# distributed-information-bottleneck/distributed-information-bottleneck.github.io

Measured on AMD Instinct MI355X. Metric: DIB train samples/sec (fwd+KL+bwd+Adam), higher is better.
Workload: dtype f32; 1 GPU; BASELINE config 3: synthetic tabular, 2^20 rows x 64 scalar features resident in HBM, posenc [2,4,8,16], encoder [128,128], E=32, integration [256,256], out=1, BCE-from-logits, Adam; per_gpu_batch=65536, global_batch=65536, parallelism=dp1, rccl_ranks_joined=1, dataset_rows=1048576, params=2224897

## Files before the change

### distributed-information-bottleneck.github.io_amd/_lib.py

```python
from __future__ import annotations

import ctypes
import os
import shutil
import subprocess
from ctypes import POINTER, c_char_p, c_float, c_int, c_int32, c_int64, c_uint32, c_uint64, c_void_p

_HERE = os.path.dirname(os.path.abspath(__file__))
CSRC = os.path.join(_HERE, "csrc")
LIB_PATH = os.path.join(_HERE, "libdib_hip.so")
LIB_OVERRIDE = os.environ.get("DIB_LIB_PATH") or None
INCLUDE_DIR = os.path.join(os.path.dirname(_HERE), "include")


def _sources() -> list:
    out = []
    for root, _, names in os.walk(CSRC):
        out += [os.path.join(root, n) for n in names if n.endswith((".h", ".hip"))]
    out += [os.path.join(INCLUDE_DIR, n) for n in os.listdir(INCLUDE_DIR) if n.endswith(".h")]
    return sorted(out)


DIB_OK = 0
ABI_VERSION = 7
ACTIVATIONS = {None: 0, "linear": 0, "None": 0, "relu": 1, "leaky_relu": 2, "tanh": 3, "sigmoid": 4, "elu": 5,
               "softplus": 6}
ACT_LEAKY_RELU_01 = 7
LOSS_KINDS = {"bce_logits": 0, "bce": 1, "sparse_cce_logits": 2, "mse": 3}
WS_U, WS_PRED, WS_ENC_OUT, WS_G_U, WS_STEP_OUT, WS_G_PRED = range(6)
WS_ENC_H0, WS_INT_H0 = 16, 32
SYNC_WORDS = 1056
FWD_DETERMINISTIC, FWD_INFERENCE, FWD_DEFER_SUMS = 1, 2, 4
HEAD_DEFER_SUMS, HEAD_NO_GRAD, HEAD_DEFER_WGRAD = 1, 2, 4
BWD_INTEGRATION_DONE = 1
TAIL_FINALIZE, TAIL_KL, TAIL_LOSS, TAIL_ADAM, TAIL_BUMP, TAIL_METRICS, TAIL_SGD, TAIL_HEAD_WGRAD, TAIL_LOSS_HEAD = \
    1, 2, 4, 8, 16, 32, 64, 128, 256
SIMILARITIES = {"l2sq": 0, "l2": 1, "l1": 2, "linf": 3, "cosine": 4}


def _hipcc() -> str:
    for cand in (shutil.which("hipcc"), "/opt/rocm/bin/hipcc"):
        if cand and os.path.exists(cand):
            return cand
    raise RuntimeError("hipcc not found: cannot build libdib_hip.so")


def _stale() -> bool:
    if not os.path.exists(LIB_PATH):
        return True
    t = os.path.getmtime(LIB_PATH)
    return any(os.path.getmtime(p) > t for p in _sources())


def build_library(force: bool = False, verbose: bool = False) -> str:
    if not force and not _stale():
        return LIB_PATH
    cmd = [_hipcc(), "--offload-arch=gfx950", "-O3", "-std=c++17", "-shared", "-fPIC",
           os.path.join(CSRC, "dib_api.hip"), "-o", LIB_PATH + f".tmp{os.getpid()}"]
    if verbose:
        print(" ".join(cmd))
    res = subprocess.run(cmd, capture_output=True, text=True)
    if res.returncode != 0:
        raise RuntimeError("hipcc failed:\n" + res.stdout + res.stderr)
    os.replace(LIB_PATH + f".tmp{os.getpid()}", LIB_PATH)
    return LIB_PATH


_lib = None

SIGNATURES = {
    "dib_version": (c_char_p, []),
    "dib_abi_version": (c_int, []),
    "dib_error_string": (c_char_p, [c_int]),
    "dib_layout_create": (c_int, [c_int, POINTER(c_int), c_int, POINTER(c_int), c_int, c_int, POINTER(c_int), c_int,
                                  c_int, c_int, c_int, c_int, POINTER(c_void_p)]),
    "dib_layout_destroy": (None, [c_void_p]),
    "dib_layout_param_count": (c_int64, [c_void_p]),
    "dib_layout_param_block": (c_int, [c_void_p, c_int, c_int, c_int, c_int, POINTER(c_int64), POINTER(c_int),
                                       POINTER(c_int)]),
    "dib_layout_table_bytes": (c_int64, [c_void_p]),
    "dib_layout_upload_tables": (c_int, [c_void_p, c_void_p, c_void_p]),
    "dib_layout_set_step_counter": (c_int, [c_void_p, c_void_p]),
    "dib_workspace_bytes": (c_int64, [c_void_p, c_int]),
    "dib_workspace_init": (c_int, [c_void_p, c_int, c_void_p, c_void_p]),
    "dib_workspace_offset": (c_int64, [c_void_p, c_int, c_int]),
    "dib_layout_wgrad_splits": (c_int, [c_void_p, c_int]),
    "dib_encoder_bank_fwd": (c_int, [c_void_p, c_void_p, c_int64, c_void_p, c_int64, c_int, c_void_p, c_uint64,
                                     c_uint32, c_int, c_void_p, c_void_p]),
    "dib_integration_fwd": (c_int, [c_void_p, c_int, c_void_p, c_void_p, c_void_p]),
    "dib_loss_fwd_bwd": (c_int, [c_void_p, c_int, c_void_p, c_int64, c_void_p, c_int64, c_int, c_float, c_int, c_void_p,
                                 c_void_p]),
    "dib_integration_bwd": (c_int, [c_void_p, c_int, c_void_p, c_void_p, c_void_p, c_void_p]),
    "dib_output_head_fused_supported": (c_int, [c_void_p, c_int]),
    "dib_integration_fwd_hidden": (c_int, [c_void_p, c_int, c_void_p, c_void_p, c_void_p]),
    "dib_output_head_fused": (c_int, [c_void_p, c_int, c_void_p, c_int64, c_void_p, c_int64, c_int, c_float, c_int, c_void_p,
                                      c_void_p, c_void_p, c_void_p]),
    "dib_integration_head_step": (c_int, [c_void_p, c_int, c_void_p, c_int64, c_void_p, c_int64, c_int, c_float, c_int, c_void_p,
                                          c_void_p, c_void_p, c_void_p]),
    "dib_integration_bwd_hidden": (c_int, [c_void_p, c_int, c_void_p, c_void_p, c_void_p, c_void_p]),
    "dib_backward": (c_int, [c_void_p, c_int, c_void_p, c_void_p, c_void_p, c_float, c_int, c_void_p, c_void_p]),
    "dib_encoder_bank_bwd": (c_int, [c_void_p, c_int, c_void_p, c_void_p, c_void_p, c_float, c_void_p, c_void_p]),
    "dib_encoder_bank_bwd_stage": (c_int, [c_void_p, c_int, c_void_p, c_void_p, c_void_p, c_float, c_int, c_void_p, c_void_p]),
    "dib_grads_finalize": (c_int, [c_void_p, c_int, c_void_p, c_void_p, c_void_p]),
    "dib_grads_finalize_part": (c_int, [c_void_p, c_int, c_int, c_void_p, c_void_p, c_void_p]),
    "dib_layout_part_range": (c_int, [c_void_p, c_int, POINTER(c_int64), POINTER(c_int64)]),
    "dib_metrics_accumulate": (c_int, [c_void_p, c_int, c_void_p, c_float, c_void_p, c_void_p, c_void_p]),
    "dib_step_tail": (c_int, [c_void_p, c_int, c_int, c_int, c_void_p, c_void_p, c_void_p, c_void_p, c_void_p, c_void_p, c_float,
                              c_float, c_float, c_float, c_void_p, c_float, c_void_p, c_void_p, c_void_p]),
    "dib_set_tuning": (c_int, [c_char_p, c_int]),
    "dib_get_tuning": (c_int, [c_char_p, POINTER(c_int)]),
    "dib_adam_step": (c_int, [c_void_p, c_void_p, c_void_p, c_void_p, c_int64, c_void_p, c_void_p, c_float, c_float,
                              c_float, c_float, c_void_p]),
    "dib_sgd_step": (c_int, [c_void_p, c_void_p, c_int64, c_void_p, c_float, c_void_p]),
    "dib_encode_deterministic": (c_int, [c_void_p, c_int, c_void_p, c_int, c_void_p, c_void_p, c_void_p, c_void_p]),
    "dib_bhattacharyya": (c_int, [c_void_p, c_void_p, c_int, c_void_p, c_void_p, c_int, c_int, c_void_p, c_void_p]),
    "dib_infonce_workspace_bytes": (c_int64, [c_int]),
    "dib_infonce_fwd_bwd": (c_int, [c_void_p, c_void_p, c_int, c_int, c_int, c_float, c_void_p, c_void_p, c_void_p, c_void_p,
                                    c_void_p]),
    "dib_positional_encoding": (c_int, [c_void_p, c_int64, c_int, c_int, c_int, c_void_p, c_void_p]),
    "dib_positional_encoding_rows": (c_int, [c_void_p, c_int64, c_void_p, c_int, c_int, c_int, c_void_p, c_void_p]),
    "dib_mlp_small_supported": (c_int, [c_void_p, c_int]),
    "dib_mlp_small_fwd": (c_int, [c_void_p, c_void_p, c_void_p, c_int64, c_void_p, c_int, c_void_p, c_void_p, c_void_p, c_void_p]),
    "dib_mlp_small_bwd": (c_int, [c_void_p, c_void_p, c_void_p, c_void_p, c_void_p, c_int, c_void_p]),
    "dib_mlp_small_head_supported": (c_int, [c_void_p, c_int]),
    "dib_mlp_small_head_workspace_bytes": (c_int64, [c_void_p, c_int]),
    "dib_mlp_small_head_step": (c_int, [c_void_p, c_void_p, c_void_p, c_int, c_void_p, c_int64, c_int, c_float, c_void_p, c_void_p,
                                        c_void_p, c_void_p, c_void_p, c_void_p, c_void_p, c_void_p, c_void_p]),
    "dib_integration_fwd_and_mlp_fwd": (c_int, [c_void_p, c_int, c_void_p, c_void_p, c_void_p, c_void_p, c_void_p, c_int64, c_void_p,
                                                c_int, c_void_p, c_void_p, c_void_p, c_void_p]),
    "dib_backward_and_mlp_bwd": (c_int, [c_void_p, c_int, c_void_p, c_void_p, c_void_p, c_float, c_int, c_void_p, c_void_p, c_void_p,
                                         c_void_p, c_void_p, c_void_p, c_int, c_void_p]),
    "dib_reduce_adam_step": (c_int, [c_void_p, c_int, c_int64, c_void_p, c_void_p, c_void_p, c_void_p, c_int64, c_void_p, c_void_p,
                                     c_float, c_float, c_float, c_float, c_void_p, c_void_p]),
    "dib_mi_workspace_bytes": (c_int64, [c_int, c_int]),
    "dib_mi_sandwich_rows": (c_int, [c_void_p, c_int, c_int, c_uint64, c_uint32, c_uint32, c_void_p, c_void_p, c_void_p,
                                     c_void_p]),
    "dib_philox_normal_fill": (c_int, [c_void_p, c_void_p, c_int64, c_int, c_int, c_int, c_uint64, c_uint32,
                                       c_void_p]),
    "dib_philox_normal_ref": (c_float, [c_uint64, c_uint32, c_uint32, c_uint32, c_uint32]),
    "dib_launch_count": (c_int64, []),
    "dib_profile_enable": (c_int, [c_int]),
    "dib_profile_summary": (c_int, [POINTER(ctypes.c_double), POINTER(c_int)]),
    "dib_profile_summary_n": (c_int, [POINTER(ctypes.c_double), POINTER(c_int), c_int]),
    "dib_gemm": (c_int, [c_int, c_int, c_int, c_int, c_void_p, c_int, c_void_p, c_int, c_void_p, c_int, c_void_p,
                         c_void_p, c_int, c_int, c_void_p, c_void_p]),
}

SIGNATURES_ST = {
    "dib_gemm_grouped": (c_int, [c_int, c_int, c_void_p, c_int, c_int, c_void_p, c_void_p, c_void_p, c_void_p, c_void_p,
                                 c_void_p, c_int, c_int, c_int, c_int64, c_void_p]),
    "dib_wgrad_grouped": (c_int, [c_int, c_void_p, c_void_p, c_int, c_int, c_int, c_void_p, c_void_p, c_void_p, c_void_p, c_int,
                                  c_int, c_int64, c_void_p]),
    "dib_reduce_splits": (c_int, [c_void_p, c_int64, c_int, c_int64, c_void_p, c_void_p]),
    "dib_reduce_splits_add": (c_int, [c_void_p, c_int64, c_int, c_int64, c_void_p, c_void_p]),
    "dib_gemm_skinny_k": (c_int, [c_int, c_int, c_void_p, c_int, c_int, c_int, c_void_p, c_void_p, c_void_p, c_void_p, c_void_p]),
    "dib_softmax_rows_fwd": (c_int, [c_void_p, c_int64, c_int, c_int, c_float, c_void_p]),
    "dib_softmax_rows_bwd": (c_int, [c_void_p, c_void_p, c_int64, c_int, c_int, c_float, c_void_p]),
    "dib_attention_stash_bytes": (c_int64, [c_int, c_int, c_int]),
    "dib_attention_fwd": (c_int, [c_void_p, c_void_p, c_void_p, c_int, c_int, c_int, c_int, c_int64, c_float, c_void_p, c_void_p,
                                  c_void_p, c_void_p]),
    "dib_attention_fwd_proj_supported": (c_int, [c_int, c_int, c_int]),
    "dib_attention_fwd_proj": (c_int, [c_void_p, c_int64, c_void_p, c_void_p, c_void_p, c_int, c_int, c_int, c_int, c_int, c_int64, c_float,
                                       c_void_p, c_void_p, c_void_p, c_void_p, c_void_p, c_void_p]),
    "dib_attention_bwd_proj": (c_int, [c_void_p, c_void_p, c_void_p, c_void_p, c_void_p, c_int, c_int, c_int, c_int, c_int, c_int64, c_float,
                                       c_void_p, c_void_p, c_void_p, c_void_p, c_void_p, c_void_p, c_int64, c_void_p]),
    "dib_attention_bwd_workspace_bytes": (c_int64, [c_int, c_int, c_int]),
    "dib_attention_bwd": (c_int, [c_void_p, c_void_p, c_void_p, c_void_p, c_void_p, c_void_p, c_void_p, c_int, c_int, c_int, c_int,
                                  c_int64, c_float, c_void_p, c_void_p, c_void_p, c_void_p, c_void_p]),
    "dib_add_layernorm_fwd": (c_int, [c_void_p, c_void_p, c_int, c_int64, c_int64, c_int, c_void_p, c_void_p, c_float, c_void_p,
                                      c_void_p, c_void_p, c_void_p]),
    "dib_add_layernorm_bwd_workspace_bytes": (c_int64, [c_int64, c_int]),
    "dib_add_layernorm_bwd": (c_int, [c_void_p, c_void_p, c_void_p, c_void_p, c_int64, c_int, c_void_p, c_void_p, c_void_p,
                                      c_void_p]),
    "dib_add_layernorm_bwd_fused": (c_int, [c_void_p, c_void_p, c_void_p, c_void_p, c_void_p, c_int64, c_int, c_void_p, c_void_p,
                                            c_int, c_void_p, c_void_p, c_void_p, c_void_p]),
    "dib_st_chain_supported": (c_int, [c_void_p, c_int64]),
    "dib_st_chain_workspace_bytes": (c_int64, [c_int64, c_int]),
    "dib_st_chain_fwd": (c_int, [c_void_p, c_int64, c_void_p, c_void_p, c_void_p, c_void_p, c_void_p, c_void_p, c_void_p, c_void_p,
                                 c_void_p, c_void_p, c_void_p]),
    "dib_st_chain_bwd": (c_int, [c_void_p, c_int64, c_void_p, c_void_p, c_int, c_int64, c_void_p, c_void_p, c_void_p, c_void_p, c_void_p,
                                 c_void_p, c_void_p, c_void_p, c_void_p, c_void_p, c_void_p]),
    "dib_mean_pool_fwd": (c_int, [c_void_p, c_int, c_int, c_int, c_void_p, c_void_p]),
    "dib_mean_pool_bwd": (c_int, [c_void_p, c_int, c_int, c_int, c_void_p, c_void_p]),
    "dib_add_inplace": (c_int, [c_void_p, c_void_p, c_int64, c_void_p]),
    "dib_act_grad_mul": (c_int, [c_void_p, c_void_p, c_int, c_int64, c_void_p, c_void_p]),
    "dib_token_kl_workspace_bytes": (c_int64, [c_int64, c_int]),
    "dib_token_reparam_kl_fwd": (c_int, [c_void_p, c_int64, c_int, c_float, c_uint64, c_uint32, c_void_p, c_int64, c_int, c_void_p,
                                         c_void_p, c_void_p, c_void_p]),
    "dib_token_reparam_kl_bwd": (c_int, [c_void_p, c_void_p, c_void_p, c_int64, c_int, c_float, c_void_p, c_float, c_void_p,
                                         c_void_p]),
    "dib_mi_probe_workspace_bytes": (c_int64, [c_int, c_int, c_int]),
    "dib_mi_probe_bounds": (c_int, [c_void_p, c_int, c_void_p, c_int, c_int, c_float, c_uint64, c_uint32, c_uint32, c_void_p,
                                    c_void_p, c_void_p, c_void_p, c_void_p]),
    "dib_loss_rows_workspace_bytes": (c_int64, [c_int]),
    "dib_loss_rows": (c_int, [c_int, c_void_p, c_int, c_void_p, c_int64, c_int, c_float, c_void_p, c_void_p, c_void_p,
                              c_void_p]),
    "dib_mi_probe_map_workspace_bytes": (c_int64, [c_int, c_int, c_int, c_int, c_int, c_int, c_int]),
    "dib_mi_probe_map": (c_int, [c_void_p, c_int, c_int, c_void_p, c_int, c_int, c_int, c_void_p, c_int, c_int, c_float, c_uint64,
                                 c_void_p, c_void_p, c_void_p, c_void_p, c_void_p, c_void_p]),
    "dib_mi_sandwich_batched_workspace_bytes": (c_int64, [c_int, c_int, c_int, c_int, c_int]),
    "dib_mi_sandwich_batched": (c_int, [c_void_p, c_int, c_int, c_int, c_void_p, c_int, c_int, c_float, c_uint64, c_uint32, c_void_p,
                                        c_void_p, c_void_p, c_void_p, c_void_p, c_void_p, c_void_p]),
}

SIGNATURES_MEASURE = {
    "dib_measure_supported": (c_int, [c_void_p]),
    "dib_measure_workspace_bytes": (c_int64, [c_void_p, c_int]),
    "dib_measure_fwd": (c_int, [c_void_p, c_void_p, c_void_p, c_int, c_uint64, c_uint32, c_float, c_float, c_void_p, c_void_p,
                                c_void_p, c_void_p, c_void_p, c_void_p, c_void_p]),
    "dib_measure_bwd": (c_int, [c_void_p, c_void_p, c_void_p, c_int, c_uint64, c_uint32, c_void_p, c_void_p, c_void_p, c_void_p,
                                c_void_p, c_int, c_void_p, c_void_p, c_void_p, c_void_p, c_void_p, c_void_p]),
    "dib_measure_symbolize": (c_int, [c_void_p, c_void_p, c_void_p, c_int64, c_void_p, c_int, c_void_p, c_void_p, c_void_p]),
    "dib_measure_posenc_rows": (c_int, [c_void_p, c_int64, c_void_p, c_int, c_int, c_int, c_int, c_void_p, c_void_p]),
}

SIGNATURES_CIRCUIT = {
    "dib_circuit_supported": (c_int, [c_int, c_int]),
    "dib_circuit_fwd": (c_int, [c_void_p, c_int, c_int, c_void_p, c_uint64, c_uint32, c_float, c_void_p, c_void_p, c_void_p,
                                c_void_p, c_void_p, c_void_p]),
    "dib_circuit_bwd": (c_int, [c_void_p, c_int, c_int, c_void_p, c_uint64, c_uint32, c_float, c_void_p, c_void_p, c_void_p,
                                c_void_p]),
    "dib_circuit_mi_workspace_bytes": (c_int64, [c_int, c_int, c_int]),
    "dib_circuit_mi_bounds": (c_int, [c_void_p, c_int, c_void_p, c_int, c_int, c_uint64, c_void_p, c_void_p, c_void_p]),
}

SIGNATURES_PARTITION = {
    "dib_partition_supported": (c_int, [c_void_p]),
    "dib_partition_symbolize": (c_int, [c_void_p, c_void_p, c_void_p, c_int, c_int64, c_int64, c_void_p, c_void_p, c_void_p,
                                        c_void_p]),
}

SIGNATURES_MI_CHANNEL = {
    "dib_mi_monte_carlo_workspace_bytes": (c_int64, [c_int, c_int, c_int, c_int, c_int]),
    "dib_mi_monte_carlo": (c_int, [c_void_p, c_int, c_int, c_int, c_void_p, c_void_p, c_int, c_int, c_uint64, c_uint32, c_void_p,
                                   c_void_p, c_void_p, c_void_p, c_void_p]),
}


def load_library(build_if_missing: bool = True):
    global _lib
    if _lib is not None:
        return _lib
    if LIB_OVERRIDE is not None:
        if not os.path.exists(LIB_OVERRIDE):
            raise RuntimeError(f"DIB_LIB_PATH={LIB_OVERRIDE} does not exist")
        return _attach(ctypes.CDLL(os.path.abspath(LIB_OVERRIDE)))
    if build_if_missing and _stale():
        try:
            build_library()
        except Exception:
            if not os.path.exists(LIB_PATH):
                raise
    if not os.path.exists(LIB_PATH):
        raise RuntimeError(f"{LIB_PATH} missing: run `python -c 'import __graft_entry__ as g; g.build()'`")
    return _attach(ctypes.CDLL(LIB_PATH))


def _attach(lib):
    global _lib
    try:
        lib.dib_abi_version.restype = c_int
        have = int(lib.dib_abi_version())
    except AttributeError:
        have = None
    if have != ABI_VERSION:
        raise RuntimeError(f"libdib_hip ABI version {have} != {ABI_VERSION} expected by this binding ({getattr(lib, '_name', '?')}): "
                           "rebuild it (python -c 'import __graft_entry__ as g; g.build()' / tools/build_variant.sh)")
    for name, (res, args) in list(SIGNATURES.items()) + list(SIGNATURES_ST.items()) + list(SIGNATURES_MEASURE.items()) \
            + list(SIGNATURES_CIRCUIT.items()) + list(SIGNATURES_PARTITION.items()) + list(SIGNATURES_MI_CHANNEL.items()):
        fn = getattr(lib, name)
        fn.restype = res
        fn.argtypes = args
    _lib = lib
    return lib


def set_tuning(key: str, value: int) -> None:
    check(load_library().dib_set_tuning(key.encode(), int(value)), f"dib_set_tuning({key})")


def get_tuning(key: str) -> int:
    v = c_int()
    check(load_library().dib_get_tuning(key.encode(), ctypes.byref(v)), f"dib_get_tuning({key})")
    return int(v.value)


class DibError(RuntimeError):
    pass


def check(code: int, what: str = "") -> None:
    if code != DIB_OK:
        msg = load_library().dib_error_string(int(code)).decode()
        raise DibError(f"libdib_hip {what} failed: {msg} (code {code})")
```

### distributed-information-bottleneck.github.io_amd/csrc/dib_api.hip

```cpp
#include <algorithm>
#include <atomic>
#include <cmath>
#include <cstdio>
#include <cstdlib>
#include <cstring>
#include <map>
#include <mutex>
#include <new>
#include <utility>
#include <vector>

#include "../../include/dib_hip.h"
#include "dib_elementwise.h"
#include "dib_gauss_lse.h"
#include "dib_mi_rows.h"
#include "dib_gemm.h"
#include "dib_wgrad_stream.h"
#include "dib_infonce_mfma.h"
#include "dib_fused.h"
#include "dib_tail.h"
#include "dib_small.h"
#include "dib_st.h"
#include "dib_attn.h"
#include "dib_attn_small.h"
#include "dib_st_chain.h"
#include "dib_measure.h"
#include "dib_circuit.h"
#include "dib_partition.h"
#include "dib_st_info.h"
#include "dib_mi_channel.h"
#include "../../include/dib_st.h"
#include "../../include/dib_measure.h"
#include "../../include/dib_circuit.h"
#include "../../include/dib_partition.h"
#include "../../include/dib_mi_channel.h"

#include "host/common.h"
#include "host/layout.h"
#include "host/gemm.h"
#include "host/encoder.h"
#include "host/small.h"
#include "host/step.h"
#include "host/infonce.h"
#include "host/st.h"
#include "host/mi.h"
#include "host/measure.h"
#include "host/circuit.h"
#include "host/partition.h"
```

### distributed-information-bottleneck.github.io_amd/csrc/host/common.h

```cpp

static std::atomic<unsigned long long> g_dib_launches{0};
#define DIB_LAUNCH(...) do { g_dib_launches.fetch_add(1, std::memory_order_relaxed); hipLaunchKernelGGL(__VA_ARGS__); } while (0)

namespace {

constexpr int64_t kAlign = 64;
constexpr int kMaxSplits = 32;
constexpr int kSmallMaxBatch = 2048;
constexpr int kSmallMaxEncWgs = 1024;
constexpr size_t kSmallMaxLds = 160 * 1024;
constexpr int kSplitRows = 512;
inline int64_t align_up(int64_t v, int64_t a = kAlign) { return (v + a - 1) / a * a; }
inline int cdiv(int64_t a, int64_t b) { return (int)((a + b - 1) / b); }
inline int grid_for(int64_t n, int per_block = 256, int cap = 256 * 16) {
  return (int)std::max<int64_t>(1, std::min<int64_t>((n + per_block - 1) / per_block, cap));
}

constexpr int kProfCats = 19;
constexpr int kProfFusedFwd = 12, kProfFusedBwd = 13, kProfOther = 14, kProfAttnFwd = 15, kProfAttnBwd = 16;
constexpr int kProfWgradStream128 = 17, kProfWgradStream64 = 18;
struct Prof {
  std::atomic<bool> on{false};
  std::mutex mu;
  std::vector<hipEvent_t> pool;
  std::vector<std::pair<hipEvent_t, hipEvent_t>> spans[kProfCats];
  hipEvent_t get() {
    if (!pool.empty()) { hipEvent_t e = pool.back(); pool.pop_back(); return e; }
    hipEvent_t e = nullptr;
    (void)hipEventCreate(&e);
    return e;
  }
} g_prof;

struct ProfScope {
  int cat; hipStream_t st; hipEvent_t a = nullptr, b = nullptr;
  ProfScope(int c, hipStream_t s) : cat(c), st(s) {
    if (g_prof.on.load(std::memory_order_relaxed) && cat != 14) {
      { std::lock_guard<std::mutex> lk(g_prof.mu); a = g_prof.get(); b = g_prof.get(); }
      (void)hipEventRecord(a, st);
    }
  }
  ~ProfScope() {
    if (a) { (void)hipEventRecord(b, st); std::lock_guard<std::mutex> lk(g_prof.mu); g_prof.spans[cat].push_back({a, b}); }
  }
};

const char* kVersion = "dib_hip 0.4 (gfx950: fused encoder-bank fwd/bwd + grouped fp32-MFMA GEMM + flash attention)";

int act_ok(int a) { return a >= 0 && a <= 7; }

struct Tuning {
  int fwd_small_wgs = 512;
  int fwd_narrow_wgs = 1024;
  int stream_rows = 8192;
  int split_policy = 1;
  int split_overhead = 128;
  int fused_encoder = 1;
  int fused_head = 1;
  int small_batch = 1;
  int small_wgs = 512;
  int mlp_row_tiles = 1;
  int infonce_one_launch = 1;
  int attn_small_bwd_waves = 8;
  int wgrad_flat_tile = 1;
  int wgrad_stream = 1;
  int wgrad_stream_rows = 8192;
  int wgrad_stream_fill = 85;
  int attn_fwd_waves = 8;
  int int_cluster_short_exchange = 1;
  int int_cluster = 8;
  int int_cluster_wgs = 256;
  int int_cluster_min_weights = 65536;
  int wgrad_max_splits = 32;
  int num_cus = 0;
};
inline Tuning& tuning() { static Tuning t; return t; }
inline const Tuning& knobs() { return tuning(); }
inline int wgrad_max_splits() { return std::max(1, std::min(32, knobs().wgrad_max_splits)); }
inline int device_cus() {
  static std::atomic<int> cus[64];
  int dev = 0;
  if (hipGetDevice(&dev) != hipSuccess || dev < 0 || dev >= 64) return 256;
  int v = cus[dev].load(std::memory_order_relaxed);
  if (v > 0) return v;
  if (hipDeviceGetAttribute(&v, hipDeviceAttributeMultiprocessorCount, dev) != hipSuccess || v <= 0) return 256;
  cus[dev].store(v, std::memory_order_relaxed);
  return v;
}
inline int split_rule_cus() { return knobs().num_cus > 0 ? knobs().num_cus : device_cus(); }

std::mutex g_attr_mu;
template <auto* Kernel>
int raise_dynamic_lds(size_t bytes) {
  if (bytes <= 64 * 1024) return DIB_OK;
  static std::atomic<size_t> granted[64];
  int dev = 0;
  std::atomic<size_t>* slot = hipGetDevice(&dev) == hipSuccess && dev >= 0 && dev < 64 ? &granted[dev] : nullptr;
  if (slot && slot->load(std::memory_order_acquire) >= bytes) return DIB_OK;
  std::lock_guard<std::mutex> lk(g_attr_mu);
  if (slot && slot->load(std::memory_order_relaxed) >= bytes) return DIB_OK;
  hipError_t e = hipFuncSetAttribute((const void*)Kernel, hipFuncAttributeMaxDynamicSharedMemorySize, (int)bytes);
  if (e != hipSuccess) return (int)e;
  if (slot) slot->store(bytes, std::memory_order_release);
  return DIB_OK;
}
template <auto* Kernel, typename... Args>
int launch_lds(dim3 grid, dim3 block, size_t lds, hipStream_t st, Args&&... args) {
  if (int rc = raise_dynamic_lds<Kernel>(lds)) return rc;
  DIB_LAUNCH(Kernel, grid, block, lds, st, std::forward<Args>(args)...);
  return (int)hipGetLastError();
}

static int* tuning_slot(const char* key) {
  Tuning& t = tuning();
  if (!key) return nullptr;
  if (!std::strcmp(key, "fwd_small_wgs")) return &t.fwd_small_wgs;
  if (!std::strcmp(key, "fwd_narrow_wgs")) return &t.fwd_narrow_wgs;
  if (!std::strcmp(key, "stream_rows")) return &t.stream_rows;
  if (!std::strcmp(key, "split_policy")) return &t.split_policy;
  if (!std::strcmp(key, "split_overhead")) return &t.split_overhead;
  if (!std::strcmp(key, "fused_encoder")) return &t.fused_encoder;
  if (!std::strcmp(key, "fused_head")) return &t.fused_head;
  if (!std::strcmp(key, "small_batch")) return &t.small_batch;
  if (!std::strcmp(key, "small_wgs")) return &t.small_wgs;
  if (!std::strcmp(key, "mlp_row_tiles")) return &t.mlp_row_tiles;
  if (!std::strcmp(key, "infonce_one_launch")) return &t.infonce_one_launch;
  if (!std::strcmp(key, "attn_small_bwd_waves")) return &t.attn_small_bwd_waves;
  if (!std::strcmp(key, "wgrad_flat_tile")) return &t.wgrad_flat_tile;
  if (!std::strcmp(key, "wgrad_stream")) return &t.wgrad_stream;
  if (!std::strcmp(key, "wgrad_stream_rows")) return &t.wgrad_stream_rows;
  if (!std::strcmp(key, "wgrad_stream_fill")) return &t.wgrad_stream_fill;
  if (!std::strcmp(key, "wgrad_max_splits")) return &t.wgrad_max_splits;
  if (!std::strcmp(key, "num_cus")) return &t.num_cus;
  if (!std::strcmp(key, "attn_fwd_waves")) return &t.attn_fwd_waves;
  if (!std::strcmp(key, "int_cluster_short_exchange")) return &t.int_cluster_short_exchange;
  if (!std::strcmp(key, "int_cluster")) return &t.int_cluster;
  if (!std::strcmp(key, "int_cluster_wgs")) return &t.int_cluster_wgs;
  if (!std::strcmp(key, "int_cluster_min_weights")) return &t.int_cluster_min_weights;
  return nullptr;
}

}

extern "C" {

const char* dib_version(void) { return kVersion; }
int dib_abi_version(void) { return DIB_ABI_VERSION; }

const char* dib_error_string(int code) {
  switch (code) {
    case DIB_OK: return "ok";
    case DIB_E_ARG: return "invalid argument";
    case DIB_E_SHAPE: return "shape mismatch";
    case DIB_E_WORKSPACE: return "workspace / descriptor tables missing";
    case DIB_E_UNSUPPORTED: return "unsupported configuration";
    case DIB_E_NODEVICE: return "no HIP device";
    default: return code > 0 ? hipGetErrorString((hipError_t)code) : "unknown dib error";
  }
}

int dib_set_tuning(const char* key, int value) {
  int* p = tuning_slot(key);
  if (!p || value < 0) return DIB_E_ARG;
  *p = value;
  return DIB_OK;
}

int dib_get_tuning(const char* key, int* value) {
  const int* p = tuning_slot(key);
  if (!p || !value) return DIB_E_ARG;
  *value = *p;
  return DIB_OK;
}

int64_t dib_launch_count(void) { return (int64_t)g_dib_launches.load(std::memory_order_relaxed); }

int dib_profile_enable(int on) {
  std::lock_guard<std::mutex> lk(g_prof.mu);
  for (int c = 0; c < kProfCats; ++c) {
    for (auto& sp : g_prof.spans[c]) { g_prof.pool.push_back(sp.first); g_prof.pool.push_back(sp.second); }
    g_prof.spans[c].clear();
  }
  g_prof.on = on != 0;
  return DIB_OK;
}

int dib_profile_summary_n(double* ms_by_category, int* launches_by_category, int n) {
  if (!ms_by_category || !launches_by_category || n < 0) return DIB_E_ARG;
  std::lock_guard<std::mutex> lk(g_prof.mu);
  for (int c = 0; c < std::min(n, kProfCats); ++c) {
    double tot = 0.0;
    for (auto& sp : g_prof.spans[c]) {
      hipError_t e = hipEventSynchronize(sp.second);
      if (e != hipSuccess) return (int)e;
      float ms = 0.f;
      e = hipEventElapsedTime(&ms, sp.first, sp.second);
      if (e != hipSuccess) return (int)e;
      tot += ms;
    }
    ms_by_category[c] = tot;
    launches_by_category[c] = (int)g_prof.spans[c].size();
  }
  for (int c = kProfCats; c < n; ++c) { ms_by_category[c] = 0.0; launches_by_category[c] = 0; }
  return DIB_OK;
}

int dib_profile_summary(double* ms_by_category, int* launches_by_category) {
  return dib_profile_summary_n(ms_by_category, launches_by_category, DIB_PROFILE_CATEGORIES);
}

}
```

### distributed-information-bottleneck.github.io_amd/csrc/host/encoder.h

```cpp

template <int H1, int H2, int E, bool RELU>
static int launch_fused_fwd(const DibFusedFwdArgs& a, int gx, int F, hipStream_t st) {
  using C = DibFusedCfg<H1, H2, E>;
  const size_t lds = (size_t)C::LDS_FLOATS * sizeof(float);
  return launch_lds<&dib_fused_encoder_fwd_kernel<H1, H2, E, RELU>>(dim3(gx, F), dim3(512), lds, st, a);
}

static int fused_gx(const dib_layout* l, int batch) { return std::max(1, std::min(cdiv(batch, 256), std::max(1, 256 / l->F))); }

static bool fused_bwd_ok(const dib_layout* l) {
  if (!(l->fused_id == 0 || l->fused_id == 1)) return false;
  for (int f = 0; f < l->F; ++f)
    if (l->in_dim[f] > 15) return false;
  return true;
}

static int fused_encoder_fwd(dib_layout* l, const dib_layout::WsMap& m, float* w, const float* x, int64_t ldx,
                             const int32_t* row_idx, int64_t row0, int batch, const float* params, uint64_t seed,
                             uint32_t step, int deterministic, hipStream_t st, int* gx_out) {
  DibFusedFwdArgs a;
  a.P = w + m.P; a.row_idx = (const int*)row_idx; a.row0 = row0; a.batch = batch; a.params = params;
  a.w_off = l->dev_fused_offs; a.b_off = l->dev_fused_offs + 3 * l->F; a.featmap = l->dev_featmap;
  a.n_blocks = l->n_blocks; a.act = l->act;
  a.h1 = w + m.enc_h[0]; a.h2 = w + m.enc_h[1]; a.enc_out = w + m.enc_out; a.U = w + m.U;
  a.kl_partial = w + m.kl_partial; a.F = l->F; a.seed = seed; a.step = step;
  a.deterministic = deterministic & DIB_FWD_DETERMINISTIC;
  a.h2mask = (unsigned long long*)(w + m.h2mask);
  a.h1mask = fused_bwd_ok(l) ? (unsigned long long*)(w + m.h1mask) : nullptr;
  if (deterministic & DIB_FWD_INFERENCE) { a.h1 = nullptr; a.h2 = nullptr; a.h2mask = nullptr; a.h1mask = nullptr; }
  a.step_dev = l->step_dev;
  const int gx = fused_gx(l, batch);
  *gx_out = gx;
  ProfScope ps(kProfFusedFwd, st);
  switch (l->fused_id) {
    case 0: return l->act == 1 ? launch_fused_fwd<128, 128, 32, true>(a, gx, l->F, st)
                                : launch_fused_fwd<128, 128, 32, false>(a, gx, l->F, st);
    case 1: return l->act == 1 ? launch_fused_fwd<32, 32, 32, true>(a, gx, l->F, st)
                                : launch_fused_fwd<32, 32, 32, false>(a, gx, l->F, st);
    case 2: return l->act == 1 ? launch_fused_fwd<32, 32, 8, true>(a, gx, l->F, st)
                                : launch_fused_fwd<32, 32, 8, false>(a, gx, l->F, st);
    case 3: return l->act == 1 ? launch_fused_fwd<64, 64, 16, true>(a, gx, l->F, st)
                                : launch_fused_fwd<64, 64, 16, false>(a, gx, l->F, st);
    default: return DIB_E_UNSUPPORTED;
  }
}

template <int H1, int H2, int E, bool RELU>
static int launch_fused_bwd(const DibFusedBwdArgs& a, int gx, int F, hipStream_t st) {
  using C = DibFusedBwdCfg<H1, H2, E>;
  const size_t lds = (size_t)C::LDS_FLOATS * sizeof(float);
  return launch_lds<&dib_fused_encoder_bwd_kernel<H1, H2, E, RELU>>(dim3(gx, F), dim3(512), lds, st, a);
}

static int fused_encoder_bwd(dib_layout* l, const dib_layout::WsMap& m, float* w, int batch, const float* params,
                             const float* beta_dev, float inv_bg, hipStream_t st) {
  DibFusedBwdArgs a;
  a.P = w + m.P; a.batch = batch; a.params = params;
  a.w_off = l->dev_fused_offs; a.b_off = l->dev_fused_offs + 3 * l->F; a.featmap = l->dev_featmap; a.act = l->act;
  a.h2mask = (const unsigned long long*)(w + m.h2mask); a.h1mask = (const unsigned long long*)(w + m.h1mask);
  a.enc_out = w + m.enc_out; a.U = w + m.U; a.GU = w + m.g_u;
  a.dout = w + m.dout; a.dh2 = w + m.g_enc_h[1]; a.dw1_partial = w + m.dw1_partial;
  a.beta_dev = beta_dev; a.inv_bg = inv_bg; a.F = l->F;
  const int gx = fused_gx(l, batch);
  ProfScope ps(kProfFusedBwd, st);
  switch (l->fused_id) {
    case 0: return l->act == 1 ? launch_fused_bwd<128, 128, 32, true>(a, gx, l->F, st)
                                : launch_fused_bwd<128, 128, 32, false>(a, gx, l->F, st);
    case 1: return l->act == 1 ? launch_fused_bwd<32, 32, 32, true>(a, gx, l->F, st)
                                : launch_fused_bwd<32, 32, 32, false>(a, gx, l->F, st);
    default: return DIB_E_UNSUPPORTED;
  }
}

static int small_tiles(int batch) { return cdiv(batch, DIB_SMALL_ROWS); }
static bool small_regime(const dib_layout* l, int batch) {
  return knobs().small_batch && batch <= kSmallMaxBatch &&
         (long long)small_tiles(batch) * l->F <= std::min(knobs().small_wgs, kSmallMaxEncWgs);
}
static bool use_small_enc(const dib_layout* l, int batch) { return l->sb_enc && small_regime(l, batch); }
static bool use_small_int(const dib_layout* l, int batch) { return l->sb_int && small_regime(l, batch); }
static int enc_dw1_parts(const dib_layout* l, int batch) {
  if (use_small_enc(l, batch)) return small_tiles(batch);
  return fused_bwd_ok(l) ? fused_gx(l, batch) * 8 : 0;
}
static int enc_kl_rows(const dib_layout* l, const dib_layout::WsMap& m, int batch) {
  if (use_small_enc(l, batch)) return small_tiles(batch);
  return l->fused_id >= 0 ? fused_gx(l, batch) * 8 : m.kl_blocks;
}

static int small_encoder_fwd(dib_layout* l, const dib_layout::WsMap& m, float* w, const float* x, int64_t ldx,
                             const int32_t* row_idx, int64_t row0, int batch, const float* params, uint64_t seed, uint32_t step,
                             int flags, hipStream_t st) {
  DibSmallEncFwdArgs a;
  a.X = x; a.ldx = ldx; a.row_idx = (const int*)row_idx; a.row0 = row0; a.batch = batch; a.params = params;
  a.w_off = l->dev_fused_offs; a.b_off = l->dev_fused_offs + 3 * l->F; a.featmap = l->dev_featmap;
  a.n_blocks = l->n_blocks; a.act = l->act; a.F = l->F; a.E = l->E; a.H1 = l->enc_units[0]; a.H2 = l->enc_units[1];
  const bool infer = (flags & DIB_FWD_INFERENCE) != 0;
  a.P = infer ? nullptr : w + m.P; a.h1 = infer ? nullptr : w + m.enc_h[0]; a.h2 = infer ? nullptr : w + m.enc_h[1];
  a.enc_out = w + m.enc_out; a.U = w + m.U; a.kl_partial = w + m.kl_partial;
  a.seed = seed; a.step = step; a.deterministic = flags & DIB_FWD_DETERMINISTIC; a.step_dev = l->step_dev;
  const size_t lds = small_encoder_lds(a.H1, a.H2, a.E, false);
  ProfScope ps(kProfOther, st);
  return launch_lds<&dib_small_encoder_fwd_kernel>(dim3(small_tiles(batch), l->F), dim3(DIB_SMALL_THREADS), lds, st, a);
}

static int small_encoder_bwd(dib_layout* l, const dib_layout::WsMap& m, float* w, int batch, const float* params,
                             const float* beta_dev, float inv_bg, hipStream_t st) {
  DibSmallEncBwdArgs a;
  a.P = w + m.P; a.batch = batch; a.params = params;
  a.w_off = l->dev_fused_offs; a.b_off = l->dev_fused_offs + 3 * l->F; a.featmap = l->dev_featmap;
  a.act = l->act; a.F = l->F; a.E = l->E; a.H1 = l->enc_units[0]; a.H2 = l->enc_units[1];
  a.h1 = w + m.enc_h[0]; a.h2 = w + m.enc_h[1]; a.enc_out = w + m.enc_out; a.U = w + m.U; a.GU = w + m.g_u;
  a.dout = w + m.dout; a.dh2 = w + m.g_enc_h[1]; a.dw1_partial = w + m.dw1_partial; a.beta_dev = beta_dev; a.inv_bg = inv_bg;
  const size_t lds = small_encoder_lds(a.H1, a.H2, a.E, true);
  ProfScope ps(kProfOther, st);
  return launch_lds<&dib_small_encoder_bwd_kernel>(dim3(small_tiles(batch), l->F), dim3(DIB_SMALL_THREADS), lds, st, a);
}

static bool use_merged_wgrad(const dib_layout* l, int batch) {
  return use_small_enc(l, batch) && use_small_int(l, batch);
}

static int encoder_chain_fwd(dib_layout* l, const dib_layout::WsMap& m, float* w, int batch, const float* params,
                             int first_group_offset, int group_count, hipStream_t st) {
  const int LE = l->n_enc + 1;
  for (int ly = 0; ly < LE; ++ly) {
    GemmCall c = l->enc_fwd[ly];
    c.first += first_group_offset;
    c.count = group_count;
    const float* A = ly == 0 ? w + m.P : w + m.enc_h[ly - 1];
    float* C = ly == LE - 1 ? w + m.enc_out : w + m.enc_h[ly];
    const int act = ly == LE - 1 ? DIB_ACT_LINEAR : l->act;
    int rc = launch_gemm<0>(l, c, A, params, C, params, nullptr, nullptr, batch, act, 1, 0, 0, st);
    if (rc) return rc;
  }
  return DIB_OK;
}

static int encoder_bank_bwd_stages(dib_layout* l, int batch, const float* params, float* grads, const float* beta_dev,
                                   float inv_global_batch, int stages, void* ws, dib_stream_t stream) {
  if (!l || !params || !grads || !beta_dev || !ws || batch <= 0 || stages < 1 || stages > 3) return DIB_E_ARG;
  if (!l->dev_groups) return DIB_E_WORKSPACE;
  hipStream_t st = (hipStream_t)stream;
  const auto m = l->map(batch);
  float* w = (float*)ws;
  float* gt = wgrad_target(m, w, grads);
  const long long sstride = align_up(l->n_params, 4);
  int rc = DIB_OK;
  const bool small = use_small_enc(l, batch);
  const bool fused = small || fused_bwd_ok(l);
  const int LE = l->n_enc + 1;
  if (stages & 1) {
    if (small) {
      rc = small_encoder_bwd(l, m, w, batch, params, beta_dev, inv_global_batch, st);
    } else if (fused) {
      rc = fused_encoder_bwd(l, m, w, batch, params, beta_dev, inv_global_batch, st);
    } else {
      { ProfScope ps(kProfOther, (hipStream_t)stream);
      DIB_LAUNCH(dib_reparam_kl_bwd_kernel, dim3(m.kl_blocks, l->F), dim3(256), 0, st, w + m.enc_out, w + m.g_u,
                         w + m.U, w + m.dout, beta_dev, inv_global_batch, batch, l->F, l->E); }
      rc = (int)hipGetLastError();
    }
    if (rc) return rc;
  }
  for (int ly = LE - 1; ly >= 0; --ly) {
    const bool last = ly == LE - 1;
    const float* gout = last ? w + m.dout : w + m.g_enc_h[ly];
    const float* hin = ly == 0 ? w + m.P : w + m.enc_h[ly - 1];
    const bool wgrad_here = (last ? (stages & 2) : (stages & 1)) && !(fused && ly == 0);
    if (wgrad_here) {
      const bool halve = l->enc_wgrad[ly].max_n <= 64 && m.nsplit >= 32 && (m.nsplit % 2) == 0;
      rc = launch_gemm<2>(l, l->enc_wgrad[ly], hin, gout, gt, nullptr, nullptr, gt, batch, 0,
                          halve ? m.nsplit / 2 : m.nsplit, halve ? 2 * m.rows_per_split : m.rows_per_split, sstride, st,
                          m.nsplit);
      if (rc) return rc;
    }
    if ((stages & 1) && ly >= 1 && !fused) {
      rc = launch_gemm<1>(l, l->enc_dgrad[ly], gout, params, w + m.g_enc_h[ly - 1], nullptr, hin, nullptr, batch,
                          l->act, 1, 0, 0, st);
      if (rc) return rc;
    }
  }
  return DIB_OK;
}

extern "C" {

int dib_encoder_bank_fwd(dib_layout* l, const float* x, int64_t ldx, const int32_t* row_idx, int64_t row0, int batch,
                         const float* params, uint64_t seed, uint32_t step, int deterministic, void* ws,
                         dib_stream_t stream) {
  if (!l || !x || !params || !ws || batch <= 0) return DIB_E_ARG;
  if (!l->dev_groups) return DIB_E_WORKSPACE;
  hipStream_t st = (hipStream_t)stream;
  const auto m = l->map(batch);
  float* w = (float*)ws;
  if (use_small_enc(l, batch)) {
    int rc = small_encoder_fwd(l, m, w, x, ldx, row_idx, row0, batch, params, seed, step, deterministic, st);
    if (rc || (deterministic & DIB_FWD_DEFER_SUMS)) return rc;
    ProfScope ps(kProfOther, st);
    DIB_LAUNCH(dib_colsum_partials_kernel, dim3(l->F), dim3(256), 0, st, w + m.kl_partial, small_tiles(batch), l->F,
                       w + m.step_out);
    return (int)hipGetLastError();
  }
  { ProfScope ps(kProfOther, (hipStream_t)stream);
  if ((long long)cdiv(l->sum_d, 64) * cdiv(batch, 64) >= 512)
    DIB_LAUNCH(dib_posenc_kernel<64>, dim3(cdiv(l->sum_d, 64), cdiv(batch, 64)), dim3(256), 0, st, x, (long long)ldx,
                       (const int*)row_idx, (long long)row0, batch, l->dev_colmap, l->sum_d, l->n_blocks, w + m.P);
  else
    DIB_LAUNCH(dib_posenc_kernel<16>, dim3(cdiv(l->sum_d, 64), cdiv(batch, 16)), dim3(256), 0, st, x, (long long)ldx,
                       (const int*)row_idx, (long long)row0, batch, l->dev_colmap, l->sum_d, l->n_blocks, w + m.P); }
  int rc = (int)hipGetLastError();
  if (rc) return rc;
  if (l->fused_id >= 0) {
    int gx = 1;
    rc = fused_encoder_fwd(l, m, w, x, ldx, row_idx, row0, batch, params, seed, step, deterministic, st, &gx);
    if (rc) return rc;
    if (deterministic & DIB_FWD_DEFER_SUMS) return DIB_OK;
    { ProfScope ps(kProfOther, (hipStream_t)stream);
    DIB_LAUNCH(dib_colsum_partials_kernel, dim3(l->F), dim3(256), 0, st, w + m.kl_partial, gx * 8, l->F,
                       w + m.step_out); }
    return (int)hipGetLastError();
  }
  rc = encoder_chain_fwd(l, m, w, batch, params, 0, l->F, st);
  if (rc) return rc;
  { ProfScope ps(kProfOther, (hipStream_t)stream);
  DIB_LAUNCH(dib_reparam_kl_fwd_kernel, dim3(m.kl_blocks, l->F), dim3(256), 0, st, w + m.enc_out, w + m.U,
                     w + m.kl_partial, (const int*)row_idx, (long long)row0, batch, l->F, l->E,
                     (unsigned long long)seed, (unsigned)step, deterministic & DIB_FWD_DETERMINISTIC, l->step_dev); }
  rc = (int)hipGetLastError();
  if (rc) return rc;
  if (deterministic & DIB_FWD_DEFER_SUMS) return DIB_OK;
  { ProfScope ps(kProfOther, (hipStream_t)stream);
  DIB_LAUNCH(dib_colsum_partials_kernel, dim3(l->F), dim3(256), 0, st, w + m.kl_partial, m.kl_blocks, l->F,
                     w + m.step_out); }
  return (int)hipGetLastError();
}

int dib_encoder_bank_bwd(dib_layout* l, int batch, const float* params, float* grads, const float* beta_dev,
                         float inv_global_batch, void* ws, dib_stream_t stream) {
  return encoder_bank_bwd_stages(l, batch, params, grads, beta_dev, inv_global_batch, 3, ws, stream);
}

int dib_encoder_bank_bwd_stage(dib_layout* l, int batch, const float* params, float* grads, const float* beta_dev,
                               float inv_global_batch, int stage, void* ws, dib_stream_t stream) {
  if (stage != 1 && stage != 2) return DIB_E_ARG;
  return encoder_bank_bwd_stages(l, batch, params, grads, beta_dev, inv_global_batch, stage, ws, stream);
}

int dib_encode_deterministic(dib_layout* l, int feature, const float* x_f, int n, const float* params, float* out,
                             void* ws, dib_stream_t stream) {
  if (!l || !x_f || !params || !out || !ws || n <= 0) return DIB_E_ARG;
  if (feature < 0 || feature >= l->F) return DIB_E_ARG;
  if (!l->dev_groups) return DIB_E_WORKSPACE;
  hipStream_t st = (hipStream_t)stream;
  const auto m = l->map(n);
  float* w = (float*)ws;
  const int d = l->dims[feature];
  { ProfScope ps(kProfOther, (hipStream_t)stream);
  DIB_LAUNCH(dib_posenc_kernel<64>, dim3(cdiv(d, 64), cdiv(n, 64)), dim3(256), 0, st, x_f, (long long)d,
                     (const int*)nullptr, 0ll, n, l->dev_colmap + l->x_off[feature], d, l->n_blocks, w + m.P); }
  int rc = (int)hipGetLastError();
  if (rc) return rc;
  rc = encoder_chain_fwd(l, m, w, n, params, feature, 1, st);
  if (rc) return rc;
  const int w2 = 2 * l->E;
  return (int)hipMemcpyAsync(out, w + m.enc_out + (int64_t)feature * n * w2, (size_t)n * w2 * sizeof(float),
                             hipMemcpyDeviceToDevice, st);
}

#ifdef DIB_FUSED_TIMING
int dib_fused_debug_read(long long* out16) {
  if (hipDeviceSynchronize() != hipSuccess) return DIB_E_ARG;
  return (int)hipMemcpyFromSymbol(out16, HIP_SYMBOL(dib_fused_dbg), 16 * sizeof(long long));
}
#endif

}
```

### distributed-information-bottleneck.github.io_amd/csrc/host/gemm.h

```cpp

namespace {

template <int MODE, int NI, int NJ, bool FLAT = false>
int launch_gemm_t(const DibGemmGroup* dev_groups, const GemmCall& c, int M, int N, const float* A, const float* B, float* C,
                  const float* bias, const float* aux, float* bias_out, int batch, int act, int nsplit,
                  int rows_per_split, long long split_stride, hipStream_t st) {
  const int tm = cdiv(M, FLAT ? 32 : 64 * NI), tn = cdiv(N, FLAT ? 256 : 64 * NJ);
  if (c.count > 65535 || (MODE == 2 && (long long)tm * tn > 65535)) return DIB_E_UNSUPPORTED;
  dim3 grid;
  if (MODE == 2) grid = dim3(nsplit, tm * tn, c.count);
  else grid = dim3(8 * cdiv(tm, 8) * tn, 1, c.count);
  constexpr int BK = FLAT ? 32 : ((NI == 2 && NJ == 2) ? 64 : ((MODE == 2 && NI == 1 && NJ == 2) ? 64 : 32));
  const long long streamed_rows = MODE == 2 ? (long long)nsplit * rows_per_split : (long long)M;
  const bool big_out = MODE != 2 && (long long)M * N * (long long)sizeof(float) * c.count >= (256ll << 20);
  const int stream_flags = streamed_rows >= knobs().stream_rows ? (big_out ? 3 : 1) : 0;
  DIB_LAUNCH((dib_gemm_kernel<MODE, NI, NJ, BK, FLAT>), grid, dim3(256), 0, st, dev_groups + c.first, A, B, C,
                     bias, aux, bias_out, batch, act, tm, tn, rows_per_split, split_stride, stream_flags);
  return (int)hipGetLastError();
}

constexpr int kWgradStreamWavesPerCu = 4;
static bool wgrad_stream_shape_ok(const DibGemmGroup* hg, int count, int batch, const float* A, const float* B, int* nt_out) {
  if (!knobs().wgrad_stream || !hg || count <= 0) return false;
  if ((((uintptr_t)A | (uintptr_t)B) & 15) != 0) return false;
  int nt = 0;
  for (int i = 0; i < count; ++i) {
    const DibGemmGroup& g = hg[i];
    const int M = g.M < 0 ? batch : g.M, N = g.N < 0 ? batch : g.N, K = g.K < 0 ? batch : g.K;
    if (M <= 0 || (M & 127) || K <= 0 || (K & 63)) return false;
    const int nt_g = N == 64 ? 2 : ((N > 0 && (N & 127) == 0) ? 4 : 0);
    if (!nt_g || (nt && nt != nt_g)) return false;
    nt = nt_g;
    if (((g.a_off + g.a_boff * batch) | (g.b_off + g.b_boff * batch) | (long long)g.lda | (long long)g.ldb) & 3) return false;
    if (g.lda < M || g.ldb < N) return false;
  }
  *nt_out = nt;
  return true;
}
static bool wgrad_stream_slabs_ok(const DibGemmGroup* hg, int count, int batch, long long tiles, int nsplit, int rows_per_split) {
  if (nsplit <= 0 || rows_per_split <= 0 || (long long)nsplit * rows_per_split < knobs().wgrad_stream_rows) return false;
  if (tiles * nsplit * 100 < (long long)knobs().wgrad_stream_fill * split_rule_cus() * kWgradStreamWavesPerCu) return false;
  for (int i = 0; i < count; ++i) {
    const int K = hg[i].K < 0 ? batch : hg[i].K;
    if ((rows_per_split & 63) && !(nsplit == 1 && rows_per_split >= K)) return false;
    if (((long long)std::min(rows_per_split, K) + 8) * std::max(hg[i].lda, hg[i].ldb) * 4 >= (1ll << 31)) return false;
  }
  return true;
}
template <int NT, int CH>
int launch_wgrad_stream(const DibGemmGroup* dev_groups, const GemmCall& c, int M, int N, const float* A, const float* B, float* C,
                        float* bias_out, int batch, int nsplit, int rows_per_split, long long split_stride, hipStream_t st) {
  const int tm = cdiv(M, 128), tn = cdiv(N, 32 * NT);
  const long long waves = (long long)tm * tn * c.count * nsplit;
  if (waves >= (1ll << 31)) return DIB_E_UNSUPPORTED;
  ProfScope ps(NT == 4 ? kProfWgradStream128 : kProfWgradStream64, st);
  const dim3 grid((unsigned)((waves + 3) / 4));
  if ((long long)nsplit * rows_per_split >= knobs().stream_rows)
    DIB_LAUNCH((dib_wgrad_stream_kernel<NT, CH, true>), grid, dim3(256), 0, st, dev_groups + c.first, A, B, C, bias_out, batch,
               c.count, tm, tn, nsplit, rows_per_split, split_stride);
  else
    DIB_LAUNCH((dib_wgrad_stream_kernel<NT, CH, false>), grid, dim3(256), 0, st, dev_groups + c.first, A, B, C, bias_out, batch,
               c.count, tm, tn, nsplit, rows_per_split, split_stride);
  return (int)hipGetLastError();
}

static void pick_wgrad_splits(long long tiles, int slots, int K, int max_splits, int* ns_out, int* rps_out) {
  const int min_rows = std::min(kSplitRows, std::max(64, *rps_out));
  const auto cost_of = [&](int ns, int rps) {
    return (double)((tiles * ns + slots - 1) / slots) * (rps + knobs().split_overhead);
  };
  {
    const long long wgs = tiles * *ns_out, rounds = (wgs + slots - 1) / slots;
    if ((double)wgs >= 0.85 * (double)(rounds * slots)) return;
  }
  double best = 1e300;
  int bns = *ns_out, brps = *rps_out;
  for (int ns = 1; ns <= max_splits; ++ns) {
    const int rps = cdiv(cdiv(K, ns), 64) * 64;
    if (ns > 1 && rps < min_rows) break;
    if (cdiv(K, rps) != ns) continue;
    const double cost = cost_of(ns, rps);
    if (cost < best) {
      best = cost;
      bns = ns;
      brps = rps;
    }
  }
  if (best >= cost_of(*ns_out, *rps_out)) return;
  *ns_out = bns;
  *rps_out = brps;
}

template <int MODE>
int launch_gemm(const DibGemmGroup* dev_groups, const GemmCall& c, const float* A, const float* B, float* C,
                const float* bias, const float* aux, float* bias_out, int batch, int act, int nsplit, int rows_per_split,
                long long split_stride, hipStream_t st, bool auto_split = false, int max_splits = 0, int* ns_used = nullptr,
                const DibGemmGroup* host_groups = nullptr) {
  if (ns_used) *ns_used = nsplit;
  if (c.count == 0) return DIB_OK;
  const int M = c.max_m < 0 ? batch : c.max_m;
  const int N = c.max_n < 0 ? batch : c.max_n;
  bool ni1 = (MODE == 2) && M <= 64, nj1 = N <= 64;
  if (MODE != 2) {
    const long long wgs = (long long)cdiv(M, 128) * cdiv(N, nj1 ? 64 : 128) * c.count;
    if (wgs < knobs().fwd_small_wgs) ni1 = true;
    if (ni1 && !nj1 && (long long)cdiv(M, 64) * cdiv(N, 128) * c.count < (MODE == 0 ? knobs().fwd_narrow_wgs : 128)) nj1 = true;
  }
  if (MODE == 2 && !ni1 && !nj1) {
    const long long wgs = (long long)cdiv(M, 128) * cdiv(N, 128) * nsplit * c.count;
    if (wgs < 256) ni1 = true;
    if (ni1 && !nj1 && (long long)cdiv(M, 64) * cdiv(N, 128) * nsplit * c.count < 128) nj1 = true;
  }
  if constexpr (MODE == 2) {
    int nt = 0;
    if (wgrad_stream_shape_ok(host_groups, c.count, batch, A, B, &nt)) {
      int ns = nsplit, rps = rows_per_split;
      const long long tiles = (long long)cdiv(M, 128) * cdiv(N, 32 * nt) * c.count;
      if (auto_split && ns > 1 && knobs().split_policy)
        pick_wgrad_splits(tiles, split_rule_cus() * kWgradStreamWavesPerCu, batch, std::max(ns, max_splits), &ns, &rps);
      if (wgrad_stream_slabs_ok(host_groups, c.count, batch, tiles, ns, rps)) {
        if (ns_used) *ns_used = ns;
        if (nt == 2) return launch_wgrad_stream<2, 4>(dev_groups, c, M, N, A, B, C, bias_out, batch, ns, rps, split_stride, st);
        return nj1 ? launch_wgrad_stream<4, 4>(dev_groups, c, M, N, A, B, C, bias_out, batch, ns, rps, split_stride, st)
                   : launch_wgrad_stream<4, 2>(dev_groups, c, M, N, A, B, C, bias_out, batch, ns, rps, split_stride, st);
      }
    }
  }
  if (MODE == 2 && auto_split && nsplit > 1 && knobs().split_policy) {
    const int per_cu = (!ni1 && !nj1) ? 2 : ((!ni1 && nj1) ? 4 : (ni1 && !nj1) ? 3 : 4);
    const long long tiles = (long long)cdiv(M, ni1 ? 64 : 128) * cdiv(N, nj1 ? 64 : 128) * c.count;
    pick_wgrad_splits(tiles, split_rule_cus() * per_cu, batch, std::max(nsplit, max_splits), &nsplit, &rows_per_split);
    if (ns_used) *ns_used = nsplit;
  }
  ProfScope ps(MODE * 4 + (ni1 ? 0 : 2) + (nj1 ? 0 : 1), st);
  if constexpr (MODE == 2) {
    if (M <= 32 && N >= 256 && knobs().wgrad_flat_tile)
      return launch_gemm_t<2, 1, 2, true>(dev_groups, c, M, N, A, B, C, bias, aux, bias_out, batch, act, nsplit, rows_per_split,
                                          split_stride, st);
  }
#define DIB_GO(NI, NJ) launch_gemm_t<MODE, NI, NJ>(dev_groups, c, M, N, A, B, C, bias, aux, bias_out, batch, act, nsplit, \
                                                   rows_per_split, split_stride, st)
  if (ni1) return nj1 ? DIB_GO(1, 1) : DIB_GO(1, 2);
  return nj1 ? DIB_GO(2, 1) : DIB_GO(2, 2);
#undef DIB_GO
}

__global__ void dib_write_desc_kernel(DibGemmGroup* dst, DibGemmGroup g) { *dst = g; }

static int retire_stale_slabs(const dib_layout* l, int batch, const DibGemmGroup* host_groups, int count, int ns, int slab_count,
                              float* gt, long long split_stride, hipStream_t st) {
  hipStreamCaptureStatus cap = hipStreamCaptureStatusNone;
  const bool capturing = hipStreamIsCapturing(st, &cap) == hipSuccess && cap == hipStreamCaptureStatusActive;
  std::lock_guard<std::mutex> lk(l->wg_mu);
  for (int i = 0; i < count; ++i) {
    const DibGemmGroup& g = host_groups[i];
    int& mark = l->slab_hwm[std::make_pair(batch, g.c_off)];
    mark = std::max(mark, ns);
    const int hwm = capturing ? std::max(mark, slab_count) : mark;
    if (ns >= hwm) continue;
    const size_t wbytes = (size_t)g.M * (size_t)g.ldc * sizeof(float);
    for (int s = ns; s < hwm; ++s) {
      hipError_t e = hipMemsetAsync(gt + (long long)s * split_stride + g.c_off, 0, wbytes, st);
      if (e == hipSuccess && g.bias_off >= 0)
        e = hipMemsetAsync(gt + (long long)s * split_stride + g.bias_off, 0, (size_t)g.N * sizeof(float), st);
      if (e != hipSuccess) return (int)e;
    }
  }
  return DIB_OK;
}

template <int MODE>
int launch_gemm(const dib_layout* l, const GemmCall& c, const float* A, const float* B, float* C, const float* bias,
                const float* aux, float* bias_out, int batch, int act, int nsplit, int rows_per_split,
                long long split_stride, hipStream_t st, int slab_count = 0) {
  int ns_used = nsplit;
  int rc = launch_gemm<MODE>(l->dev_groups, c, A, B, C, bias, aux, bias_out, batch, act, nsplit, rows_per_split, split_stride,
                             st, MODE == 2, slab_count, &ns_used, MODE == 2 ? l->table.data() + c.first : nullptr);
  if (MODE == 2 && rc == DIB_OK && slab_count > 1)
    rc = retire_stale_slabs(l, batch, l->table.data() + c.first, c.count, ns_used, slab_count, C, split_stride, st);
  return rc;
}

}

static int merged_wgrad(dib_layout* l, const dib_layout::WsMap& m, float* w, int batch, float* gt, int first, int count,
                        hipStream_t st) {
  if (count <= 0) return DIB_OK;
  const auto& host = wg_table_host(l, m, batch);
  GemmCall c;
  c.first = 0; c.count = count;
  for (int i = first; i < first + count; ++i) { c.max_m = std::max(c.max_m, host[i].M); c.max_n = std::max(c.max_n, host[i].N); }
  const DibGemmGroup* dev = reinterpret_cast<const DibGemmGroup*>(w + m.wg_table) + first;
  int ns_used = m.nsplit;
  int rc = launch_gemm<2>(dev, c, w, w, gt, nullptr, nullptr, gt, batch, 0, m.nsplit, m.rows_per_split, align_up(l->n_params, 4), st,
                          true, m.nsplit, &ns_used, host.data() + first);
  if (rc == DIB_OK && m.nsplit > 1)
    rc = retire_stale_slabs(l, batch, host.data() + first, count, ns_used, m.nsplit, gt, align_up(l->n_params, 4), st);
  return rc;
}

extern "C" {

int dib_gemm(int mode, int M, int N, int K, const float* A, int lda, const float* B, int ldb, float* C, int ldc,
             const float* bias, const float* aux, int ldaux, int act, void* dev_desc, dib_stream_t stream) {
  if (!A || !B || !C || !dev_desc || M <= 0 || N <= 0 || K <= 0 || mode < 0 || mode > 2) return DIB_E_ARG;
  hipStream_t st = (hipStream_t)stream;
  DibGemmGroup g = make_group(Off(), lda, Off(), ldb, Off(), ldc, bias ? 0 : -1, Off(), ldaux, M, N, K);
  if ((((uintptr_t)A | (uintptr_t)B) & 15) != 0) return DIB_E_ARG;
  DIB_LAUNCH(dib_write_desc_kernel, dim3(1), dim3(1), 0, st, (DibGemmGroup*)dev_desc, g);
  if (hipError_t e = hipGetLastError(); e != hipSuccess) return (int)e;
  const int tm = cdiv(M, 128), tn = cdiv(N, 128);
  const DibGemmGroup* dg = (const DibGemmGroup*)dev_desc;
  const dim3 g1(8 * cdiv(tm, 8) * tn, 1, 1);
  if (mode == 0)
    DIB_LAUNCH((dib_gemm_kernel<0, 2, 2, 32>), g1, dim3(256), 0, st, dg, A, B, C, bias, aux, (float*)nullptr, 0,
                       act, tm, tn, 0, 0ll);
  else if (mode == 1)
    DIB_LAUNCH((dib_gemm_kernel<1, 2, 2, 32>), g1, dim3(256), 0, st, dg, A, B, C, bias, aux, (float*)nullptr, 0,
                       act, tm, tn, 0, 0ll);
  else
    DIB_LAUNCH((dib_gemm_kernel<2, 2, 2, 32>), dim3(1, tm * tn, 1), dim3(256), 0, st, dg, A, B, C,
                       (const float*)nullptr, aux, (float*)bias, 0, act, tm, tn, K, 0ll);
  return (int)hipGetLastError();
}

static_assert(sizeof(dib_gemm_desc) == sizeof(DibGemmGroup), "public descriptor must mirror the kernel's group struct");

int dib_gemm_grouped(int mode, int n_groups, const dib_gemm_desc* dev_desc, int max_m, int max_n, const float* A,
                     const float* B, float* C, const float* bias, const float* aux, float* bias_out, int act, int nsplit,
                     int rows_per_split, int64_t split_stride, dib_stream_t stream) {
  if (!dev_desc || !A || !B || !C || n_groups <= 0 || max_m <= 0 || max_n <= 0 || mode < 0 || mode > 2 || !act_ok(act))
    return DIB_E_ARG;
  if (mode == 2 && (nsplit <= 0 || rows_per_split <= 0)) return DIB_E_ARG;
  GemmCall c;
  c.first = 0; c.count = n_groups; c.max_m = max_m; c.max_n = max_n;
  const DibGemmGroup* g = reinterpret_cast<const DibGemmGroup*>(dev_desc);
  hipStream_t st = (hipStream_t)stream;
  switch (mode) {
    case 0: return launch_gemm<0>(g, c, A, B, C, bias, aux, nullptr, 0, act, 1, 0, 0, st);
    case 1: return launch_gemm<1>(g, c, A, B, C, nullptr, aux, nullptr, 0, act, 1, 0, 0, st);
    default: return launch_gemm<2>(g, c, A, B, C, nullptr, nullptr, bias_out, 0, 0, nsplit, rows_per_split,
                                   (long long)split_stride, st);
  }
}

int dib_wgrad_grouped(int n_groups, const dib_gemm_desc* dev_desc, const dib_gemm_desc* host_desc, int max_m, int max_n, int batch,
                      const float* A, const float* B, float* C, float* bias_out, int nsplit, int rows_per_split,
                      int64_t split_stride, dib_stream_t stream) {
  if (!dev_desc || !host_desc || !A || !B || !C || n_groups <= 0 || max_m <= 0 || max_n <= 0 || batch < 0 || nsplit <= 0 ||
      rows_per_split <= 0)
    return DIB_E_ARG;
  GemmCall c;
  c.first = 0; c.count = n_groups; c.max_m = max_m; c.max_n = max_n;
  return launch_gemm<2>(reinterpret_cast<const DibGemmGroup*>(dev_desc), c, A, B, C, nullptr, nullptr, bias_out, batch, 0, nsplit,
                        rows_per_split, (long long)split_stride, (hipStream_t)stream, false, 0, nullptr,
                        reinterpret_cast<const DibGemmGroup*>(host_desc));
}

int dib_gemm_skinny_k(int mode, int n_groups, const dib_gemm_desc* dev_desc, int M, int N, int K, const float* A,
                      const float* B, float* C, const float* bias, dib_stream_t stream) {
  if (!dev_desc || !A || !B || !C || n_groups <= 0 || M <= 0 || N <= 0 || K <= 0 || mode < 0 || mode > 1) return DIB_E_ARG;
  if (K > 32 || (K & 3) || (N & 31) || n_groups > 65535 || cdiv(N, 128) > 65535) return DIB_E_UNSUPPORTED;
  const DibGemmGroup* g = reinterpret_cast<const DibGemmGroup*>(dev_desc);
  const int total_tiles = cdiv(M, 64), cn = cdiv(N, 128);
  int chunks = std::max(1, std::min(total_tiles, cdiv(4096, cn * n_groups)));
  int tiles = std::min(8, cdiv(total_tiles, chunks));
  chunks = cdiv(total_tiles, tiles);
  const int nt_store = (long long)M * N * (long long)sizeof(float) * n_groups >= (256ll << 20) ? 1 : 0;
  const dim3 grid(chunks, cn, n_groups);
  hipStream_t st = (hipStream_t)stream;
  if (mode == 0)
    DIB_LAUNCH(dib_gemm_skinnyk_kernel<0>, grid, dim3(256), 0, st, g, A, B, C, bias, M, N, K, tiles, nt_store);
  else
    DIB_LAUNCH(dib_gemm_skinnyk_kernel<1>, grid, dim3(256), 0, st, g, A, B, C, (const float*)nullptr, M, N, K, tiles,
                       nt_store);
  return (int)hipGetLastError();
}

int dib_reduce_splits(const float* partial, int64_t n, int nsplit, int64_t stride, float* out, dib_stream_t stream) {
  if (!partial || !out || n <= 0 || nsplit <= 0 || (n & 3) || (stride & 3)) return DIB_E_ARG;
  DIB_LAUNCH(dib_reduce_splits_kernel, dim3(grid_for(n / 4)), dim3(256), 0, (hipStream_t)stream, partial,
                     (long long)n, nsplit, (long long)stride, out, (const float*)nullptr);
  return (int)hipGetLastError();
}

int dib_reduce_splits_add(const float* partial, int64_t n, int nsplit, int64_t stride, float* out, dib_stream_t stream) {
  if (!partial || !out || n <= 0 || nsplit <= 0 || (n & 3) || (stride & 3)) return DIB_E_ARG;
  DIB_LAUNCH(dib_reduce_splits_kernel, dim3(grid_for(n / 4)), dim3(256), 0, (hipStream_t)stream, partial,
                     (long long)n, nsplit, (long long)stride, out, (const float*)out);
  return (int)hipGetLastError();
}

}
```

### distributed-information-bottleneck.github.io_amd/csrc/host/layout.h

```cpp

namespace {

struct GemmCall {
  int first = 0, count = 0;
  int max_m = 0, max_n = 0;
};

struct Off { int64_t fixed = 0, per_batch = 0; };
inline Off fixed_off(int64_t o) { Off r; r.fixed = o; return r; }
inline Off batch_off(int64_t o) { Off r; r.per_batch = o; return r; }

DibGemmGroup make_group(Off a, int lda, Off b, int ldb, Off c, int ldc, int64_t bias_off, Off aux, int ldaux, int M,
                        int N, int K) {
  DibGemmGroup g;
  std::memset(&g, 0, sizeof(g));
  g.a_off = a.fixed; g.a_boff = a.per_batch; g.b_off = b.fixed; g.b_boff = b.per_batch;
  g.c_off = c.fixed; g.c_boff = c.per_batch; g.aux_off = aux.fixed; g.aux_boff = aux.per_batch;
  g.bias_off = bias_off;
  g.M = M; g.N = N; g.K = K; g.lda = lda; g.ldb = ldb; g.ldc = ldc; g.ldaux = ldaux;
  return g;
}

}

struct dib_layout {
  int F = 0, n_enc = 0, E = 0, n_int = 0, out_dim = 0, use_pe = 0, n_freq = 0, act = 0, out_act = 0;
  std::vector<int> dims, enc_units, int_units;
  int sum_d = 0, pw = 0, n_blocks = 1;
  std::vector<int> in_dim, in_off, x_off;
  std::vector<int> enc_width;
  std::vector<int> int_width;
  int64_t n_params = 0;
  long long max_wgrad_tiles64 = 0;
  std::vector<std::vector<int64_t>> enc_w_off, enc_b_off;
  std::vector<int64_t> int_w_off, int_b_off;
  std::vector<DibGemmGroup> table;
  std::vector<int4> colmap;
  std::vector<GemmCall> enc_fwd, enc_dgrad, enc_wgrad, int_fwd, int_dgrad, int_wgrad;
  const DibGemmGroup* dev_groups = nullptr;
  const int4* dev_colmap = nullptr;
  int fused_id = -1;
  std::vector<long long> fused_offs;
  std::vector<int4> featmap;
  const long long* dev_fused_offs = nullptr;
  const int4* dev_featmap = nullptr;
  const unsigned* step_dev = nullptr;
  bool sb_enc = false, sb_int = false;
  int sb_int_lds = 0;
  int wg_groups() const { return n_enc * F + n_int + 1; }
  mutable std::map<int, std::vector<DibGemmGroup>> wg_tables;
  mutable std::mutex wg_mu;
  mutable std::map<std::pair<int, long long>, int> slab_hwm;

  struct WsMap {
    int64_t P, enc_out, U, pred, g_pred, g_u, dout;
    std::vector<int64_t> enc_h, int_h, g_enc_h, g_int_h;
    int64_t step_out, kl_partial, loss_partial, wgrad_partial, dw1_partial, h2mask, h1mask, skinny_partial, sync, wg_table, total;
    int64_t cl_sync; std::vector<int64_t> cl_x;
    int skinny_chunks, skinny_rows;
    int kl_blocks, loss_blocks, nsplit, rows_per_split;
  };
  WsMap map(int B) const {
    WsMap m;
    int64_t o = 0;
    auto take = [&](int64_t nfloats) { int64_t r = o; o = align_up(o + nfloats); return r; };
    m.P = take((int64_t)B * pw);
    for (int l = 0; l < n_enc; ++l) m.enc_h.push_back(take((int64_t)B * F * enc_units[l]));
    m.enc_out = take((int64_t)B * F * 2 * E);
    m.U = take((int64_t)B * F * E);
    for (int l = 0; l < n_int; ++l) m.int_h.push_back(take((int64_t)B * int_units[l]));
    m.pred = take((int64_t)B * out_dim);
    m.g_pred = take((int64_t)B * out_dim);
    for (int l = 0; l < n_int; ++l) m.g_int_h.push_back(take((int64_t)B * int_units[l]));
    m.g_u = take((int64_t)B * F * E);
    m.dout = take((int64_t)B * F * 2 * E);
    for (int l = 0; l < n_enc; ++l) m.g_enc_h.push_back(take((int64_t)B * F * enc_units[l]));
    m.step_out = take(F + 3);
    const int E4 = (E + 3) / 4;
    const int rpb = std::max(1, 256 / E4);
    m.kl_blocks = cdiv(B, rpb);
    m.kl_partial = take((int64_t)std::max(m.kl_blocks, 8 * 256) * F);
    m.loss_blocks = cdiv(B, 256);
    m.loss_partial = take((int64_t)std::max(m.loss_blocks, 512) * 2);
    int ns = std::min(std::min(kMaxSplits, wgrad_max_splits()), std::max(1, B / kSplitRows));
    if (B >= 256 && max_wgrad_tiles64 * ns < 256) ns = std::min(std::min(kMaxSplits, wgrad_max_splits()), std::max(ns, B / 128));
    int rps = cdiv(cdiv(B, ns), 32) * 32;
    ns = cdiv(B, rps);
    m.nsplit = ns;
    m.rows_per_split = rps;
    m.wgrad_partial = take(ns > 1 ? (int64_t)ns * align_up(n_params, 4) : 0);
    m.dw1_partial = take(std::max<int64_t>(fused_id >= 0 && n_enc == 2 ? (int64_t)cdiv(256, F) * 8 * F * 16 * enc_units[0] : 0,
                                           sb_enc && B <= kSmallMaxBatch && (int64_t)cdiv(B, DIB_SMALL_ROWS) * F <= kSmallMaxEncWgs
                                               ? (int64_t)cdiv(B, DIB_SMALL_ROWS) * F * 16 * enc_units[0] : 0));
    m.h2mask = take(fused_id >= 0 ? (int64_t)F * B * 4 : 0);
    m.h1mask = take(fused_id >= 0 ? (int64_t)F * B * 4 : 0);
    m.skinny_rows = std::max(B <= 2048 ? 16 : 64, cdiv(B, 512));
    m.skinny_chunks = cdiv(B, m.skinny_rows);
    {
      const int win = n_int == 0 ? F * E : int_units[n_int - 1];
      m.skinny_partial = take(out_dim <= 8 ? (int64_t)m.skinny_chunks * ((int64_t)win * out_dim + out_dim) : 0);
    }
    m.sync = take(DIB_TAIL_SYNC_WORDS);
    m.wg_table = take((int64_t)wg_groups() * (int64_t)(sizeof(DibGemmGroup) / sizeof(float)));
    const bool cl_ok = sb_int && B <= kSmallMaxBatch;
    m.cl_sync = take(cl_ok ? 2ll * cdiv(B, DIB_SMALL_ROWS) * DIB_SMALL_CL_SYNC_WORDS : 0);
    for (int l = 0; l < n_int; ++l) m.cl_x.push_back(take(cl_ok ? (int64_t)B * int_units[l] : 0));
    m.total = o;
    return m;
  }
};

static size_t small_encoder_lds(int H1, int H2, int E, bool bwd) {
  const int k = bwd ? 2 : 1;
  return (size_t)DIB_SMALL_ROWS * (20 + k * dib_small_pitch(H1) + k * dib_small_pitch(H2) + dib_small_pitch(2 * E)) * sizeof(float) +
         (size_t)DIB_SMALL_XCH_FLOATS_WIDE * sizeof(float);
}

static const std::vector<DibGemmGroup>& wg_table_host(const dib_layout* l, const dib_layout::WsMap& m, int batch) {
  std::lock_guard<std::mutex> lk(l->wg_mu);
  auto it = l->wg_tables.find(batch);
  if (it != l->wg_tables.end()) return it->second;
  std::vector<DibGemmGroup> t;
  const int64_t B = batch;
  for (int ly = 1; ly <= l->n_enc; ++ly) {
    const int win = l->enc_width[ly - 1], wout = l->enc_width[ly];
    for (int f = 0; f < l->F; ++f)
      t.push_back(make_group(fixed_off(m.enc_h[ly - 1] + (int64_t)f * win * B), win,
                             fixed_off((ly == l->n_enc ? m.dout : m.g_enc_h[ly]) + (int64_t)f * wout * B), wout,
                             fixed_off(l->enc_w_off[ly][f]), wout, l->enc_b_off[ly][f], Off(), 0, win, wout, -1));
  }
  for (int ly = 0; ly <= l->n_int; ++ly) {
    const int win = ly == 0 ? l->F * l->E : l->int_width[ly - 1], wout = l->int_width[ly];
    t.push_back(make_group(fixed_off(ly == 0 ? m.U : m.int_h[ly - 1]), win, fixed_off(ly == l->n_int ? m.g_pred : m.g_int_h[ly]), wout,
                           fixed_off(l->int_w_off[ly]), wout, l->int_b_off[ly], Off(), 0, win, wout, -1));
  }
  return l->wg_tables.emplace(batch, std::move(t)).first->second;
}

static inline float* wgrad_target(const dib_layout::WsMap& m, float* w, float* grads) {
  return m.nsplit > 1 ? w + m.wgrad_partial : grads;
}

static void part_bounds(const dib_layout* l, int part, long long* beg, long long* end) {
  const long long split = l->int_w_off[0], tail = l->enc_w_off[l->n_enc][0], all = l->n_params;
  switch (part) {
    case 0: *beg = 0; *end = split; break;
    case 1: *beg = split; *end = all; break;
    case 2: *beg = 0; *end = tail; break;
    case 3: *beg = tail; *end = split; break;
    default: *beg = 0; *end = all; break;
  }
}

extern "C" {

int dib_layout_create(int F, const int* feature_dims, int n_enc, const int* enc_units, int E, int n_int,
                      const int* int_units, int out_dim, int use_pe, int n_freq, int act, int out_act,
                      dib_layout** out) {
  if (!out || F <= 0 || !feature_dims || n_enc < 0 || n_int < 0 || E <= 0 || out_dim <= 0) return DIB_E_ARG;
  if ((n_enc > 0 && !enc_units) || (n_int > 0 && !int_units)) return DIB_E_ARG;
  if (!act_ok(act) || !act_ok(out_act)) return DIB_E_UNSUPPORTED;
  if ((E + 3) / 4 > 256) return DIB_E_UNSUPPORTED;
  dib_layout* l = new (std::nothrow) dib_layout();
  if (!l) return DIB_E_ARG;
  l->F = F; l->n_enc = n_enc; l->E = E; l->n_int = n_int; l->out_dim = out_dim;
  l->use_pe = use_pe ? 1 : 0; l->n_freq = n_freq; l->act = act; l->out_act = out_act;
  l->dims.assign(feature_dims, feature_dims + F);
  l->enc_units.assign(enc_units, enc_units + n_enc);
  l->int_units.assign(int_units, int_units + n_int);
  l->n_blocks = (l->use_pe && n_freq > 1) ? n_freq : 1;
  for (int f = 0; f < F; ++f) {
    if (l->dims[f] <= 0) { delete l; return DIB_E_ARG; }
    l->x_off.push_back(l->sum_d);
    l->in_off.push_back(l->pw);
    l->in_dim.push_back(l->dims[f] * l->n_blocks);
    l->sum_d += l->dims[f];
    l->pw += l->dims[f] * l->n_blocks;
    for (int c = 0; c < l->dims[f]; ++c) l->colmap.push_back(make_int4(f, c, l->dims[f], l->in_off[f]));
  }
  for (int i = 0; i < n_enc; ++i) { if (enc_units[i] <= 0) { delete l; return DIB_E_ARG; } l->enc_width.push_back(enc_units[i]); }
  l->enc_width.push_back(2 * E);
  for (int i = 0; i < n_int; ++i) { if (int_units[i] <= 0) { delete l; return DIB_E_ARG; } l->int_width.push_back(int_units[i]); }
  l->int_width.push_back(out_dim);

  int64_t o = 0;
  const int LE = n_enc + 1, LI = n_int + 1;
  l->enc_w_off.assign(LE, std::vector<int64_t>(F));
  l->enc_b_off.assign(LE, std::vector<int64_t>(F));
  for (int ly = 0; ly < LE; ++ly) {
    const int wout = l->enc_width[ly];
    for (int f = 0; f < F; ++f) {
      const int win = ly == 0 ? l->in_dim[f] : l->enc_width[ly - 1];
      o = align_up(o, 4);
      l->enc_w_off[ly][f] = o;
      o += (int64_t)win * wout;
    }
    o = align_up(o, 4);
    for (int f = 0; f < F; ++f) { l->enc_b_off[ly][f] = o; o += wout; }
  }
  for (int ly = 0; ly < LI; ++ly) {
    const int win = ly == 0 ? F * E : l->int_width[ly - 1];
    const int wout = l->int_width[ly];
    o = align_up(o, 4);
    l->int_w_off.push_back(o);
    o += (int64_t)win * wout;
    o = align_up(o, 4);
    l->int_b_off.push_back(o);
    o += wout;
  }
  l->n_params = o;

  auto& T = l->table;
  for (int ly = 0; ly < LE; ++ly) {
    const int wout = l->enc_width[ly];
    GemmCall fw, dg, wg;
    fw.first = (int)T.size();
    for (int f = 0; f < F; ++f) {
      const int win = ly == 0 ? l->in_dim[f] : l->enc_width[ly - 1];
      const Off a = batch_off(ly == 0 ? (int64_t)l->in_off[f] : (int64_t)f * win);
      T.push_back(make_group(a, win, fixed_off(l->enc_w_off[ly][f]), wout, batch_off((int64_t)f * wout), wout,
                             l->enc_b_off[ly][f], Off(), 0, -1, wout, win));
    }
    fw.count = F; fw.max_m = -1; fw.max_n = wout;
    l->enc_fwd.push_back(fw);
    dg.first = (int)T.size();
    if (ly >= 1) {
      const int win = l->enc_width[ly - 1];
      for (int f = 0; f < F; ++f)
        T.push_back(make_group(batch_off((int64_t)f * wout), wout, fixed_off(l->enc_w_off[ly][f]), wout,
                               batch_off((int64_t)f * win), win, -1, batch_off((int64_t)f * win), win, -1, win, wout));
      dg.count = F; dg.max_m = -1; dg.max_n = win;
    }
    l->enc_dgrad.push_back(dg);
    wg.first = (int)T.size();
    int max_in = 0;
    for (int f = 0; f < F; ++f) {
      const int win = ly == 0 ? l->in_dim[f] : l->enc_width[ly - 1];
      const Off a = batch_off(ly == 0 ? (int64_t)l->in_off[f] : (int64_t)f * win);
      T.push_back(make_group(a, win, batch_off((int64_t)f * wout), wout, fixed_off(l->enc_w_off[ly][f]), wout,
                             l->enc_b_off[ly][f], Off(), 0, win, wout, -1));
      max_in = std::max(max_in, win);
    }
    wg.count = F; wg.max_m = max_in; wg.max_n = wout;
    l->max_wgrad_tiles64 = std::max(l->max_wgrad_tiles64, (long long)cdiv(max_in, 64) * cdiv(wout, 64) * F);
    l->enc_wgrad.push_back(wg);
  }
  for (int ly = 0; ly < LI; ++ly) {
    const int win = ly == 0 ? F * E : l->int_width[ly - 1];
    const int wout = l->int_width[ly];
    GemmCall fw, dg, wg;
    fw.first = (int)T.size();
    T.push_back(make_group(Off(), win, fixed_off(l->int_w_off[ly]), wout, Off(), wout, l->int_b_off[ly], Off(), 0, -1,
                           wout, win));
    fw.count = 1; fw.max_m = -1; fw.max_n = wout;
    l->int_fwd.push_back(fw);
    dg.first = (int)T.size();
    T.push_back(make_group(Off(), wout, fixed_off(l->int_w_off[ly]), wout, Off(), win, -1, Off(), win, -1, win, wout));
    dg.count = 1; dg.max_m = -1; dg.max_n = win;
    l->int_dgrad.push_back(dg);
    wg.first = (int)T.size();
    T.push_back(make_group(Off(), win, Off(), wout, fixed_off(l->int_w_off[ly]), wout, l->int_b_off[ly], Off(), 0, win,
                           wout, -1));
    wg.count = 1; wg.max_m = win; wg.max_n = wout;
    l->max_wgrad_tiles64 = std::max(l->max_wgrad_tiles64, (long long)cdiv(win, 64) * cdiv(wout, 64));
    l->int_wgrad.push_back(wg);
  }
  {
    static const int kFused[][3] = {{128, 128, 32}, {32, 32, 32}, {32, 32, 8}, {64, 64, 16}};
    bool in_ok = true;
    for (int f = 0; f < F; ++f) in_ok = in_ok && l->in_dim[f] <= 16;
    if (knobs().fused_encoder && n_enc == 2 && in_ok && act >= 0 && act <= 2)
      for (int i = 0; i < 4; ++i)
        if (kFused[i][0] == enc_units[0] && kFused[i][1] == enc_units[1] && kFused[i][2] == E) l->fused_id = i;
    for (int ly = 0; ly < LE && ly < 3; ++ly)
      for (int f = 0; f < F; ++f) l->fused_offs.push_back(l->enc_w_off[ly][f]);
    for (int ly = LE; ly < 3; ++ly)
      for (int f = 0; f < F; ++f) l->fused_offs.push_back(0);
    for (int ly = 0; ly < LE && ly < 3; ++ly)
      for (int f = 0; f < F; ++f) l->fused_offs.push_back(l->enc_b_off[ly][f]);
    for (int ly = LE; ly < 3; ++ly)
      for (int f = 0; f < F; ++f) l->fused_offs.push_back(0);
    for (int f = 0; f < F; ++f) l->featmap.push_back(make_int4(l->dims[f], l->in_dim[f], l->x_off[f], l->in_off[f]));
  }
  {
    bool in_ok = true;
    for (int f = 0; f < F; ++f) in_ok = in_ok && l->in_dim[f] <= 15;
    const bool pl_act = act >= 0 && act <= 2 && out_act >= 0 && out_act <= 2;
    l->sb_enc = pl_act && n_enc == 2 && in_ok && enc_units[0] % 16 == 0 && enc_units[1] % 16 == 0 && (2 * E) % 16 == 0 &&
                enc_units[0] <= 1024 && enc_units[1] <= 1024 && E <= 512 &&
                small_encoder_lds(enc_units[0], enc_units[1], E, false) <= kSmallMaxLds &&
                small_encoder_lds(enc_units[0], enc_units[1], E, true) <= kSmallMaxLds;
    bool w_ok = n_int >= 1 && n_int <= 3 && (F * E) % 16 == 0;
    int64_t fl = (int64_t)DIB_SMALL_ROWS * dib_small_pitch(F * E);
    for (int i = 0; i < n_int && w_ok; ++i) {
      w_ok = int_units[i] % 16 == 0 && int_units[i] <= 1024;
      fl += 2ll * DIB_SMALL_ROWS * dib_small_pitch(int_units[i]);
    }
    fl += (int64_t)DIB_SMALL_ROWS * dib_small_pitch(out_dim) + DIB_SMALL_XCH_FLOATS + (w_ok ? 9 * (int_units[n_int - 1] + 1) + 32 : 0);
    l->sb_int = pl_act && w_ok && fl * 4 <= 150 * 1024;
    l->sb_int_lds = (int)(fl * 4);
  }
  *out = l;
  return DIB_OK;
}

void dib_layout_destroy(dib_layout* l) {
  if (!l) return;
  delete l;
}

int64_t dib_layout_param_count(const dib_layout* l) { return l ? l->n_params : DIB_E_ARG; }

int dib_layout_param_block(const dib_layout* l, int net, int layer, int feature, int what, int64_t* offset,
                           int* rows, int* cols) {
  if (!l || !offset || !rows || !cols) return DIB_E_ARG;
  if (net == 0) {
    if (layer < 0 || layer > l->n_enc || feature < 0 || feature >= l->F) return DIB_E_ARG;
    const int win = layer == 0 ? l->in_dim[feature] : l->enc_width[layer - 1];
    const int wout = l->enc_width[layer];
    if (what == 0) { *offset = l->enc_w_off[layer][feature]; *rows = win; *cols = wout; }
    else { *offset = l->enc_b_off[layer][feature]; *rows = 1; *cols = wout; }
    return DIB_OK;
  }
  if (net == 1) {
    if (layer < 0 || layer > l->n_int) return DIB_E_ARG;
    const int win = layer == 0 ? l->F * l->E : l->int_width[layer - 1];
    const int wout = l->int_width[layer];
    if (what == 0) { *offset = l->int_w_off[layer]; *rows = win; *cols = wout; }
    else { *offset = l->int_b_off[layer]; *rows = 1; *cols = wout; }
    return DIB_OK;
  }
  return DIB_E_ARG;
}

int64_t dib_layout_table_bytes(const dib_layout* l) {
  if (!l) return DIB_E_ARG;
  return align_up((int64_t)l->table.size() * sizeof(DibGemmGroup), 256) +
         align_up((int64_t)l->colmap.size() * sizeof(int4), 256) +
         align_up((int64_t)l->fused_offs.size() * sizeof(long long), 256) +
         align_up((int64_t)l->featmap.size() * sizeof(int4), 256);
}

int dib_layout_upload_tables(dib_layout* l, void* dev_tables, dib_stream_t stream) {
  if (!l || !dev_tables) return DIB_E_ARG;
  hipStream_t st = (hipStream_t)stream;
  const int64_t gbytes = (int64_t)l->table.size() * sizeof(DibGemmGroup);
  char* base = (char*)dev_tables;
  hipError_t e = hipMemcpyAsync(base, l->table.data(), gbytes, hipMemcpyHostToDevice, st);
  if (e != hipSuccess) return (int)e;
  char* cm = base + align_up(gbytes, 256);
  e = hipMemcpyAsync(cm, l->colmap.data(), l->colmap.size() * sizeof(int4), hipMemcpyHostToDevice, st);
  if (e != hipSuccess) return (int)e;
  char* fo = cm + align_up((int64_t)l->colmap.size() * sizeof(int4), 256);
  e = hipMemcpyAsync(fo, l->fused_offs.data(), l->fused_offs.size() * sizeof(long long), hipMemcpyHostToDevice, st);
  if (e != hipSuccess) return (int)e;
  char* fmp = fo + align_up((int64_t)l->fused_offs.size() * sizeof(long long), 256);
  e = hipMemcpyAsync(fmp, l->featmap.data(), l->featmap.size() * sizeof(int4), hipMemcpyHostToDevice, st);
  if (e != hipSuccess) return (int)e;
  l->dev_groups = (const DibGemmGroup*)base;
  l->dev_colmap = (const int4*)cm;
  l->dev_fused_offs = (const long long*)fo;
  l->dev_featmap = (const int4*)fmp;
  return DIB_OK;
}

int dib_layout_set_step_counter(dib_layout* l, const uint32_t* step_dev) {
  if (!l) return DIB_E_ARG;
  l->step_dev = (const unsigned*)step_dev;
  return DIB_OK;
}

int64_t dib_workspace_bytes(const dib_layout* l, int batch) {
  if (!l || batch <= 0) return DIB_E_ARG;
  return l->map(batch).total * (int64_t)sizeof(float);
}

int dib_workspace_init(const dib_layout* l, int batch, void* ws, dib_stream_t stream) {
  if (!l || !ws || batch <= 0) return DIB_E_ARG;
  const auto m = l->map(batch);
  hipError_t e0 = hipMemsetAsync((float*)ws + m.sync, 0, (size_t)DIB_TAIL_SYNC_WORDS * sizeof(unsigned), (hipStream_t)stream);
  if (e0 != hipSuccess) return (int)e0;
  if (l->sb_int && batch <= kSmallMaxBatch) {
    e0 = hipMemsetAsync((float*)ws + m.cl_sync, 0, 2 * (size_t)cdiv(batch, DIB_SMALL_ROWS) * DIB_SMALL_CL_SYNC_WORDS * sizeof(unsigned),
                        (hipStream_t)stream);
    if (e0 != hipSuccess) return (int)e0;
  }
  {
    const auto& t = wg_table_host(l, m, batch);
    e0 = hipMemcpyAsync((float*)ws + m.wg_table, t.data(), t.size() * sizeof(DibGemmGroup), hipMemcpyHostToDevice, (hipStream_t)stream);
    if (e0 != hipSuccess) return (int)e0;
  }
  e0 = hipMemsetAsync((float*)ws + m.step_out, 0, (size_t)(l->F + 3) * sizeof(float), (hipStream_t)stream);
  if (e0 != hipSuccess) return (int)e0;
  if (m.nsplit <= 1) return DIB_OK;
  return (int)hipMemsetAsync((float*)ws + m.wgrad_partial, 0,
                             (size_t)m.nsplit * (size_t)align_up(l->n_params, 4) * sizeof(float), (hipStream_t)stream);
}

int64_t dib_workspace_offset(const dib_layout* l, int batch, int which) {
  if (!l || batch <= 0) return DIB_E_ARG;
  const auto m = l->map(batch);
  int64_t o = -1;
  switch (which) {
    case DIB_WS_U: o = m.U; break;
    case DIB_WS_PRED: o = m.pred; break;
    case DIB_WS_ENC_OUT: o = m.enc_out; break;
    case DIB_WS_G_U: o = m.g_u; break;
    case DIB_WS_STEP_OUT: o = m.step_out; break;
    case DIB_WS_G_PRED: o = m.g_pred; break;
    default:
      if (which >= DIB_WS_ENC_H0 && which < DIB_WS_ENC_H0 + l->n_enc) o = m.enc_h[which - DIB_WS_ENC_H0];
      else if (which >= DIB_WS_INT_H0 && which < DIB_WS_INT_H0 + l->n_int) o = m.int_h[which - DIB_WS_INT_H0];
      else return DIB_E_ARG;
  }
  return o * (int64_t)sizeof(float);
}

int dib_layout_wgrad_splits(const dib_layout* l, int batch) {
  if (!l || batch <= 0) return DIB_E_ARG;
  return l->map(batch).nsplit;
}

int dib_layout_part_range(const dib_layout* l, int part, int64_t* offset, int64_t* count) {
  if (!l || !offset || !count || part < 0 || part > 3) return DIB_E_ARG;
  long long beg, end;
  part_bounds(l, part, &beg, &end);
  *offset = beg;
  *count = end - beg;
  return DIB_OK;
}

}
```

### distributed-information-bottleneck.github.io_amd/engine.py

```python
from __future__ import annotations

import ctypes
import math
from ctypes import byref, c_int, c_int64, c_void_p
from typing import Dict, List, Optional, Sequence

import numpy as np
import torch

from . import _lib
from ._lib import ACTIVATIONS, LOSS_KINDS, check
from .utils import mi_sandwich_rows


def _ptr(t: Optional[torch.Tensor]):
    return c_void_p(t.data_ptr()) if t is not None else c_void_p(0)


class HipEngine:

    def __init__(self, feature_dimensionalities: Sequence[int], feature_encoder_architecture: Sequence[int],
                 integration_network_architecture: Sequence[int], output_dimensionality: int,
                 use_positional_encoding: bool = True, number_positional_encoding_frequencies: int = 5,
                 activation_fn: Optional[str] = "relu", feature_embedding_dimension: int = 32,
                 output_activation_fn: Optional[str] = None, device: Optional[str] = None, init_seed: int = 0):
        if not torch.cuda.is_available():
            raise RuntimeError("HipEngine needs an AMD GPU (torch.cuda.is_available() is False); "
                               "the Distributed-IB path has no CPU fallback")
        self.lib = _lib.load_library()
        if activation_fn not in ACTIVATIONS or output_activation_fn not in ACTIVATIONS:
            raise ValueError(f"unsupported activation {activation_fn!r}/{output_activation_fn!r}; "
                             f"supported: {sorted(k for k in ACTIVATIONS if isinstance(k, str))}")
        self.device = torch.device(device or f"cuda:{torch.cuda.current_device()}")
        self.F = len(feature_dimensionalities)
        self.E = int(feature_embedding_dimension)
        self.dims = [int(d) for d in feature_dimensionalities]
        self.sum_d = sum(self.dims)
        self.out_dim = int(output_dimensionality)
        self.enc_units = [int(u) for u in feature_encoder_architecture]
        self.int_units = [int(u) for u in integration_network_architecture]
        ci = lambda xs: (c_int * max(1, len(xs)))(*xs)
        handle = c_void_p()
        check(self.lib.dib_layout_create(self.F, ci(self.dims), len(self.enc_units), ci(self.enc_units), self.E,
                                         len(self.int_units), ci(self.int_units), self.out_dim,
                                         1 if use_positional_encoding else 0,
                                         int(number_positional_encoding_frequencies), ACTIVATIONS[activation_fn],
                                         ACTIVATIONS[output_activation_fn], byref(handle)), "dib_layout_create")
        self.layout = handle
        self.n_params = int(self.lib.dib_layout_param_count(self.layout))
        n_alloc = (self.n_params + 3) // 4 * 4
        with torch.cuda.device(self.device):
            z = lambda n, dt=torch.float32: torch.zeros(n, dtype=dt, device=self.device)
            self.params, self.grads, self.adam_m, self.adam_v = z(n_alloc), z(n_alloc), z(n_alloc), z(n_alloc)
            self.beta_dev = torch.ones(1, dtype=torch.float32, device=self.device)
            self.lr_dev = torch.full((1,), 1e-3, dtype=torch.float32, device=self.device)
            self._lr_host: Optional[float] = 1e-3
            self.t_dev = z(1, torch.int64)
            self._metrics_stride = (self.F + 3 + 3) // 4 * 4
            self._metrics2 = z(2 * self._metrics_stride)
            self.metrics_acc = self._metrics2[: self.F + 3]
            self.metrics_acc_val = self._metrics2[self._metrics_stride: self._metrics_stride + self.F + 3]
            tb = int(self.lib.dib_layout_table_bytes(self.layout))
            self._tables = torch.zeros(tb, dtype=torch.uint8, device=self.device)
            check(self.lib.dib_layout_upload_tables(self.layout, _ptr(self._tables), self._stream()),
                  "dib_layout_upload_tables")
            torch.cuda.synchronize(self.device)
        self._ws: Dict[int, torch.Tensor] = {}
        self._ws_pinned = set()
        self._ws_gen: Dict[int, int] = {}
        self._scratch: Optional[torch.Tensor] = None
        self._fused_head: Dict[int, bool] = {}
        self._infonce_ws: Dict[int, torch.Tensor] = {}
        self.blocks = self._query_blocks()
        self.set_flat_params(self.glorot_uniform(init_seed))

    def _stream(self):
        return c_void_p(torch.cuda.current_stream(self.device).cuda_stream)

    def __del__(self):
        try:
            if getattr(self, "layout", None):
                self.lib.dib_layout_destroy(self.layout)
                self.layout = None
        except Exception:
            pass

    _WS_KEEP = 4

    def workspace(self, batch: int) -> torch.Tensor:
        ws = self._ws.pop(batch, None)
        if ws is None:
            nbytes = int(self.lib.dib_workspace_bytes(self.layout, batch))
            if nbytes <= 0:
                raise _lib.DibError(f"dib_workspace_bytes({batch}) -> {nbytes}")
            ws = torch.empty(nbytes // 4, dtype=torch.float32, device=self.device)
            check(self.lib.dib_workspace_init(self.layout, batch, _ptr(ws), self._stream()), "dib_workspace_init")
            unpinned = [b for b in self._ws if b not in self._ws_pinned]
            while len(unpinned) >= self._WS_KEEP:
                self._ws.pop(unpinned.pop(0))
            self._ws_gen[batch] = self._ws_gen.get(batch, 0) + 1
        self._ws[batch] = ws
        return ws

    def scratch(self, nbytes: int) -> torch.Tensor:
        n = (int(nbytes) + 3) // 4
        if self._scratch is None or self._scratch.numel() < n:
            self._scratch = torch.empty(n, dtype=torch.float32, device=self.device)
        return self._scratch

    def ws_view(self, batch: int, which: int, numel: int) -> torch.Tensor:
        off = int(self.lib.dib_workspace_offset(self.layout, batch, which))
        if off < 0:
            raise _lib.DibError(f"dib_workspace_offset -> {off}")
        return self.workspace(batch)[off // 4: off // 4 + numel]

    def _query_blocks(self) -> List[dict]:
        out = []
        off, rows, cols = c_int64(), c_int(), c_int()
        for net, nl in ((0, len(self.enc_units) + 1), (1, len(self.int_units) + 1)):
            for layer in range(nl):
                for f in (range(self.F) if net == 0 else [0]):
                    for what in (0, 1):
                        check(self.lib.dib_layout_param_block(self.layout, net, layer, f, what, byref(off), byref(rows),
                                                              byref(cols)), "dib_layout_param_block")
                        out.append(dict(net=net, layer=layer, feature=f, what=what, offset=off.value, rows=rows.value,
                                        cols=cols.value))
        return out

    def glorot_uniform(self, seed: int) -> np.ndarray:
        rng = np.random.default_rng(seed)
        flat = np.zeros(self.params.numel(), dtype=np.float32)
        for b in self.blocks:
            if b["what"] == 0:
                lim = math.sqrt(6.0 / (b["rows"] + b["cols"]))
                n = b["rows"] * b["cols"]
                flat[b["offset"]: b["offset"] + n] = rng.uniform(-lim, lim, size=n).astype(np.float32)
        return flat

    def set_flat_params(self, flat: np.ndarray) -> None:
        flat = np.asarray(flat, dtype=np.float32).reshape(-1)
        buf = np.zeros(self.params.numel(), dtype=np.float32)
        buf[: min(len(flat), len(buf))] = flat[: len(buf)]
        self.params.copy_(torch.from_numpy(buf))

    def get_flat_params(self) -> np.ndarray:
        return self.params.detach().cpu().numpy().copy()

    def get_flat_grads(self) -> np.ndarray:
        return self.grads.detach().cpu().numpy().copy()

    def reset_optimizer(self) -> None:
        self.adam_m.zero_()
        self.adam_v.zero_()
        self.t_dev.zero_()

    def set_beta(self, v: float) -> None:
        self.beta_dev.fill_(float(v))

    def get_beta(self) -> float:
        return float(self.beta_dev.item())

    def set_lr(self, v: float) -> None:
        if self._lr_host != float(v):
            self.lr_dev.fill_(float(v))
            self._lr_host = float(v)

    def invalidate_lr_cache(self) -> None:
        self._lr_host = None

    def to_device(self, a, dtype=torch.float32) -> torch.Tensor:
        if isinstance(a, torch.Tensor):
            return a.to(device=self.device, dtype=dtype).contiguous()
        return torch.from_numpy(np.ascontiguousarray(np.asarray(a))).to(device=self.device, dtype=dtype).contiguous()

    def forward(self, x: torch.Tensor, row_idx: Optional[torch.Tensor], row0: int, batch: int, seed: int, step: int,
                deterministic: bool = False, inference: bool = False, hidden_only: bool = False,
                defer_sums: bool = False, companion=None) -> None:
        self.encoder_forward(x, row_idx, row0, batch, seed, step, deterministic, inference, defer_sums)
        ws, st = self.workspace(batch), self._stream()
        if companion is not None:
            assert not hidden_only
            check(self.lib.dib_integration_fwd_and_mlp_fwd(self.layout, batch, _ptr(self.params), _ptr(ws), *companion, st),
                  "dib_integration_fwd_and_mlp_fwd")
        elif hidden_only:
            check(self.lib.dib_integration_fwd_hidden(self.layout, batch, _ptr(self.params), _ptr(ws), st),
                  "dib_integration_fwd_hidden")
        else:
            check(self.lib.dib_integration_fwd(self.layout, batch, _ptr(self.params), _ptr(ws), st), "dib_integration_fwd")

    def encoder_forward(self, x: torch.Tensor, row_idx: Optional[torch.Tensor], row0: int, batch: int, seed: int, step: int,
                        deterministic: bool = False, inference: bool = False, defer_sums: bool = False) -> None:
        ws = self.workspace(batch)
        self._ws_gen[batch] += 1
        check(self.lib.dib_encoder_bank_fwd(self.layout, _ptr(x), x.stride(0), _ptr(row_idx), int(row0), batch,
                                            _ptr(self.params), int(seed), int(step) & 0xFFFFFFFF,
                                            (_lib.FWD_DETERMINISTIC if deterministic else 0) | (_lib.FWD_INFERENCE if inference else 0)
                                            | (_lib.FWD_DEFER_SUMS if defer_sums else 0), _ptr(ws), self._stream()),
              "dib_encoder_bank_fwd")

    def loss(self, loss_kind: str, y: torch.Tensor, row_idx, row0: int, batch: int, inv_global_batch: float,
             defer_sums: bool = False) -> None:
        ws = self.workspace(batch)
        check(self.lib.dib_loss_fwd_bwd(self.layout, LOSS_KINDS[loss_kind], _ptr(y), y.stride(0), _ptr(row_idx),
                                        int(row0), batch, float(inv_global_batch), _lib.HEAD_DEFER_SUMS if defer_sums else 0,
                                        _ptr(ws), self._stream()),
              "dib_loss_fwd_bwd")

    def step_tail(self, batch: int, part: int, flags: int, inv_global_batch: float = 0.0, optimizer=None,
                  grad_scale: float = 1.0, metrics_acc: Optional[torch.Tensor] = None) -> None:
        b1, b2, eps = 0.9, 0.999, 1e-7
        if optimizer is not None:
            if optimizer[0] == "adam":
                flags |= _lib.TAIL_ADAM
                b1, b2, eps = (float(v) for v in optimizer[1:4])
            elif optimizer[0] == "sgd":
                flags |= _lib.TAIL_SGD
            else:
                raise ValueError(f"optimizer {optimizer[0]!r}")
        check(self.lib.dib_step_tail(self.layout, batch, int(part), int(flags), _ptr(self.params), _ptr(self.grads),
                                     _ptr(self.adam_m), _ptr(self.adam_v), _ptr(self.lr_dev), _ptr(self.t_dev), b1, b2, eps,
                                     float(grad_scale), _ptr(self.beta_dev), float(inv_global_batch),
                                     _ptr(self.metrics_acc if metrics_acc is None else metrics_acc),
                                     _ptr(self.workspace(batch)), self._stream()), "dib_step_tail")

    def optimizer_step_part(self, batch: int, part: int, optimizer, bump: bool) -> None:
        self.step_tail(batch, part, _lib.TAIL_BUMP if (bump and optimizer[0] == "adam") else 0, optimizer=optimizer)

    def part_range(self, part: int):
        off, cnt = c_int64(), c_int64()
        check(self.lib.dib_layout_part_range(self.layout, part, byref(off), byref(cnt)), "dib_layout_part_range")
        return off.value, cnt.value

    def backward(self, row_idx, row0: int, batch: int, seed: int, step: int, inv_global_batch: float,
                 on_integration_grads_ready=None, hidden_only: bool = False, on_encoder_front_grads_ready=None,
                 finish_flags: int = 0, optimizer=None, integration_done: bool = False, companion=None,
                 metrics_acc: Optional[torch.Tensor] = None) -> None:
        ws = self.workspace(batch)
        st = self._stream()
        FIN = _lib.TAIL_FINALIZE
        head = _lib.TAIL_HEAD_WGRAD if hidden_only else 0
        if on_integration_grads_ready is None and (integration_done or not hidden_only):
            assert on_encoder_front_grads_ready is None
            bflags = _lib.BWD_INTEGRATION_DONE if integration_done else 0
            if companion is not None:
                check(self.lib.dib_backward_and_mlp_bwd(self.layout, batch, _ptr(self.params), _ptr(self.grads), _ptr(self.beta_dev),
                                                        float(inv_global_batch), bflags, _ptr(ws), *companion, st),
                      "dib_backward_and_mlp_bwd")
            else:
                check(self.lib.dib_backward(self.layout, batch, _ptr(self.params), _ptr(self.grads), _ptr(self.beta_dev),
                                            float(inv_global_batch), bflags, _ptr(ws), st), "dib_backward")
            self.step_tail(batch, -1, FIN | head | finish_flags | (_lib.TAIL_BUMP if optimizer and optimizer[0] == "adam" else 0),
                           inv_global_batch, optimizer=optimizer, metrics_acc=metrics_acc)
            return
        assert companion is None, "a companion pass rides on dib_backward (no bucket hooks)"
        if not integration_done:
            fn = self.lib.dib_integration_bwd_hidden if hidden_only else self.lib.dib_integration_bwd
            check(fn(self.layout, batch, _ptr(self.params), _ptr(self.grads), _ptr(ws), st), "dib_integration_bwd")
        if on_integration_grads_ready is not None:
            assert optimizer is None, "the data-parallel caller steps the optimizer after its all-reduces"
            self.step_tail(batch, 1, FIN | head)
            off, cnt = self.part_range(1)
            on_integration_grads_ready(self.grads[off: off + cnt])
        if on_encoder_front_grads_ready is not None:
            assert on_integration_grads_ready is not None, "the three-bucket protocol needs both hooks"
            for stage, part in ((1, 2), (2, 3)):
                check(self.lib.dib_encoder_bank_bwd_stage(self.layout, batch, _ptr(self.params), _ptr(self.grads),
                                                          _ptr(self.beta_dev), float(inv_global_batch), stage, _ptr(ws), st),
                      "dib_encoder_bank_bwd_stage")
                self.step_tail(batch, part, FIN | (finish_flags if stage == 2 else 0), inv_global_batch, metrics_acc=metrics_acc)
                if stage == 1:
                    off, cnt = self.part_range(2)
                    on_encoder_front_grads_ready(self.grads[off: off + cnt])
            return
        check(self.lib.dib_encoder_bank_bwd(self.layout, batch, _ptr(self.params), _ptr(self.grads),
                                            _ptr(self.beta_dev), float(inv_global_batch), _ptr(ws), st), "dib_encoder_bank_bwd")
        if on_integration_grads_ready is not None:
            self.step_tail(batch, 0, FIN | finish_flags, inv_global_batch, metrics_acc=metrics_acc)
        else:
            self.step_tail(batch, -1, FIN | head | finish_flags | (_lib.TAIL_BUMP if optimizer and optimizer[0] == "adam" else 0),
                           inv_global_batch, optimizer=optimizer, metrics_acc=metrics_acc)

    def accumulate_metrics(self, batch: int, inv_global_batch: float) -> None:
        check(self.lib.dib_metrics_accumulate(self.layout, batch, _ptr(self.beta_dev), float(inv_global_batch),
                                              _ptr(self.metrics_acc), _ptr(self.workspace(batch)), self._stream()),
              "dib_metrics_accumulate")

    def _head_fused(self, kind: int) -> bool:
        fused_head = self._fused_head.get(kind)
        if fused_head is None:
            fused_head = self._fused_head[kind] = bool(self.lib.dib_output_head_fused_supported(self.layout, kind))
        return fused_head

    fused_optimizer_tail = True

    def train_step(self, x, y, row_idx, row0: int, batch: int, seed: int, step: int, loss_kind: str,
                   inv_global_batch: Optional[float] = None, accumulate: bool = True,
                   on_integration_grads_ready=None, on_encoder_front_grads_ready=None, optimizer=None) -> None:
        inv = 1.0 / batch if inv_global_batch is None else inv_global_batch
        kind = LOSS_KINDS[loss_kind]
        fused_head = self._head_fused(kind)
        finish = _lib.TAIL_KL | (_lib.TAIL_LOSS_HEAD if fused_head else _lib.TAIL_LOSS) | (_lib.TAIL_METRICS if accumulate else 0)
        if fused_head:
            self.encoder_forward(x, row_idx, row0, batch, seed, step, defer_sums=True)
            single = on_integration_grads_ready is None
            check(self.lib.dib_integration_head_step(self.layout, kind, _ptr(y), y.stride(0), _ptr(row_idx), int(row0), batch,
                                                     float(inv), _lib.HEAD_DEFER_SUMS | (_lib.HEAD_DEFER_WGRAD if single else 0),
                                                     _ptr(self.params), _ptr(self.grads),
                                                     _ptr(self.workspace(batch)), self._stream()), "dib_integration_head_step")
            self.backward(row_idx, row0, batch, seed, step, inv, on_integration_grads_ready, hidden_only=True,
                          on_encoder_front_grads_ready=on_encoder_front_grads_ready, finish_flags=finish, optimizer=optimizer,
                          integration_done=True)
            return
        self.forward(x, row_idx, row0, batch, seed, step, defer_sums=True)
        self.loss(loss_kind, y, row_idx, row0, batch, inv, defer_sums=True)
        self.backward(row_idx, row0, batch, seed, step, inv, on_integration_grads_ready, hidden_only=False,
                      on_encoder_front_grads_ready=on_encoder_front_grads_ready, finish_flags=finish, optimizer=optimizer)

    def eval_step(self, x, y, row_idx, row0: int, batch: int, seed: int, step: int, loss_kind: str,
                  inv_global_batch: Optional[float] = None, metrics_acc: Optional[torch.Tensor] = None) -> None:
        inv = 1.0 / batch if inv_global_batch is None else inv_global_batch
        kind = LOSS_KINDS[loss_kind]
        fused_head = self._head_fused(kind)
        if fused_head:
            self.encoder_forward(x, row_idx, row0, batch, seed, step, inference=True, defer_sums=True)
            check(self.lib.dib_integration_head_step(self.layout, kind, _ptr(y), y.stride(0), _ptr(row_idx), int(row0), batch,
                                                     float(inv), _lib.HEAD_DEFER_SUMS | _lib.HEAD_NO_GRAD, _ptr(self.params), None,
                                                     _ptr(self.workspace(batch)), self._stream()), "dib_integration_head_step")
        else:
            self.forward(x, row_idx, row0, batch, seed, step, inference=True, defer_sums=True)
            self.loss(loss_kind, y, row_idx, row0, batch, inv, defer_sums=True)
        self.step_tail(batch, -1, _lib.TAIL_KL | (_lib.TAIL_LOSS_HEAD if fused_head else _lib.TAIL_LOSS) | _lib.TAIL_METRICS, inv,
                       metrics_acc=metrics_acc)

    def enable_step_counter(self, value: int = 0) -> None:
        if getattr(self, "step_dev", None) is None:
            self.step_dev = torch.zeros(1, dtype=torch.int32, device=self.device)
            check(self.lib.dib_layout_set_step_counter(self.layout, _ptr(self.step_dev)), "dib_layout_set_step_counter")
        self.set_step_counter(value)

    def set_step_counter(self, value: int) -> None:
        v = int(value) & 0xFFFFFFFF
        self.step_dev.fill_(v - (1 << 32) if v >= (1 << 31) else v)

    def capture_step_graph(self, x, y, batch: int, loss_kind: str, inv_global_batch: float, seed: int, train: bool,
                           optimizer: str = "adam", opt_args=(0.9, 0.999, 1e-7)):
        assert getattr(self, "step_dev", None) is not None, "call enable_step_counter() first"
        idx_stage = torch.zeros(batch, dtype=torch.int32, device=self.device)
        self.workspace(batch)
        self._ws_pinned.add(batch)
        saved = [t.clone() for t in (self.metrics_acc, self.grads, self.params, self.adam_m, self.adam_v, self.t_dev,
                                     self.step_dev)]

        def body():
            if train:
                self.train_step(x, y, idx_stage, 0, batch, seed, 0, loss_kind, inv_global_batch,
                                optimizer=("adam", *opt_args) if optimizer == "adam" else ("sgd",))
            else:
                self.eval_step(x, y, idx_stage, 0, batch, seed, 0, loss_kind, inv_global_batch)
            self.step_dev.add_(1)

        def restore():
            for t, v in zip((self.metrics_acc, self.grads, self.params, self.adam_m, self.adam_v, self.t_dev, self.step_dev),
                            saved):
                t.copy_(v)

        body()
        restore()
        torch.cuda.synchronize(self.device)
        graph = torch.cuda.CUDAGraph()
        with torch.cuda.graph(graph):
            body()
        restore()
        return graph, idx_stage

    def release_step_graph(self, batch: int) -> None:
        self._ws_pinned.discard(batch)
        unpinned = [b for b in self._ws if b not in self._ws_pinned]
        while len(unpinned) > self._WS_KEEP:
            self._ws.pop(unpinned.pop(0))

    def adam_step(self, beta1=0.9, beta2=0.999, eps=1e-7, grad_scale=1.0) -> None:
        check(self.lib.dib_adam_step(_ptr(self.params), _ptr(self.grads), _ptr(self.adam_m), _ptr(self.adam_v),
                                     self.n_params, _ptr(self.lr_dev), _ptr(self.t_dev), beta1, beta2, eps,
                                     float(grad_scale), self._stream()), "dib_adam_step")

    def sgd_step(self, grad_scale=1.0) -> None:
        check(self.lib.dib_sgd_step(_ptr(self.params), _ptr(self.grads), self.n_params, _ptr(self.lr_dev),
                                    float(grad_scale), self._stream()), "dib_sgd_step")

    def read_metrics(self, reset: bool = True) -> np.ndarray:
        m = self.metrics_acc.detach().cpu().numpy().astype(np.float64)
        if reset:
            self.metrics_acc.zero_()
        return m

    def read_metrics_pair(self, reset: bool = True):
        both = self._metrics2.detach().cpu().numpy().astype(np.float64)
        if reset:
            self._metrics2.zero_()
        n, st = self.F + 3, self._metrics_stride
        return both[:n].copy(), both[st: st + n].copy()

    def profile_enable(self, on: bool) -> None:
        check(self.lib.dib_profile_enable(1 if on else 0), "dib_profile_enable")

    def profile_summary(self) -> dict:
        return profile_summary(self.lib)


    def pred(self, batch: int) -> torch.Tensor:
        return self.ws_view(batch, _lib.WS_PRED, batch * self.out_dim).view(batch, self.out_dim)

    def u(self, batch: int) -> torch.Tensor:
        return self.ws_view(batch, _lib.WS_U, batch * self.F * self.E).view(batch, self.F * self.E)

    def enc_out(self, batch: int) -> torch.Tensor:
        return self.ws_view(batch, _lib.WS_ENC_OUT, batch * self.F * 2 * self.E).view(self.F, batch, 2 * self.E) \
            .permute(1, 0, 2)

    def enc_h(self, batch: int, layer: int) -> torch.Tensor:
        w = self.enc_units[layer]
        return self.ws_view(batch, _lib.WS_ENC_H0 + layer, batch * self.F * w).view(self.F, batch, w)

    def int_h(self, batch: int, layer: int) -> torch.Tensor:
        w = self.int_units[layer]
        return self.ws_view(batch, _lib.WS_INT_H0 + layer, batch * w).view(batch, w)

    def g_u(self, batch: int) -> torch.Tensor:
        return self.ws_view(batch, _lib.WS_G_U, batch * self.F * self.E).view(batch, self.F * self.E)

    def g_pred(self, batch: int) -> torch.Tensor:
        return self.ws_view(batch, _lib.WS_G_PRED, batch * self.out_dim).view(batch, self.out_dim)

    def step_out(self, batch: int) -> torch.Tensor:
        return self.ws_view(batch, _lib.WS_STEP_OUT, self.F + 3)

    def encode_feature(self, f: int, x_f) -> torch.Tensor:
        xf = self.to_device(x_f).reshape(-1, self.dims[f])
        n = xf.shape[0]
        out = torch.empty((n, 2 * self.E), dtype=torch.float32, device=self.device)
        ws = self.scratch(int(self.lib.dib_workspace_bytes(self.layout, n)))
        check(self.lib.dib_encode_deterministic(self.layout, int(f), _ptr(xf), n, _ptr(self.params), _ptr(out),
                                                _ptr(ws), self._stream()), "dib_encode_deterministic")
        return out

    def bhattacharyya(self, mu1, lv1, mu2, lv2) -> torch.Tensor:
        mu1, lv1, mu2, lv2 = [self.to_device(t) for t in (mu1, lv1, mu2, lv2)]
        n, d = mu1.shape
        m = mu2.shape[0]
        out = torch.empty((n, m), dtype=torch.float32, device=self.device)
        check(self.lib.dib_bhattacharyya(_ptr(mu1), _ptr(lv1), n, _ptr(mu2), _ptr(lv2), m, d, _ptr(out),
                                         self._stream()), "dib_bhattacharyya")
        return out

    def infonce(self, emb_x: torch.Tensor, emb_y: torch.Tensor, similarity: str = "l2", temperature: float = 1.0,
                want_grads: bool = True, out_gx: Optional[torch.Tensor] = None, out_gy: Optional[torch.Tensor] = None,
                loss_out: Optional[torch.Tensor] = None):
        emb_x, emb_y = emb_x.contiguous(), emb_y.contiguous()
        b, d = emb_x.shape
        ws = self._infonce_ws.get(b)
        if ws is None:
            if len(self._infonce_ws) >= 4:
                self._infonce_ws.pop(next(iter(self._infonce_ws)))
            ws = self._infonce_ws[b] = torch.empty(int(self.lib.dib_infonce_workspace_bytes(b)) // 4, dtype=torch.float32,
                                                   device=self.device)
        loss = loss_out if loss_out is not None else torch.empty(1, dtype=torch.float32, device=self.device)
        assert loss.numel() == 1 and loss.dtype == torch.float32 and loss.device == self.device
        gx = gy = None
        if want_grads:
            for o in (out_gx, out_gy):
                assert o is None or (o.is_contiguous() and tuple(o.shape) == (b, d) and o.dtype == torch.float32)
            gx = out_gx if out_gx is not None else torch.empty_like(emb_x)
            gy = out_gy if out_gy is not None else torch.empty_like(emb_y)
        check(self.lib.dib_infonce_fwd_bwd(_ptr(emb_x), _ptr(emb_y), b, d, _lib.SIMILARITIES[similarity], float(temperature),
                                           _ptr(gx), _ptr(gy), _ptr(loss), _ptr(ws), self._stream()), "dib_infonce_fwd_bwd")
        return loss, gx, gy

    def backward_from_pred_grad(self, g_pred: torch.Tensor, row_idx, row0: int, batch: int, seed: int, step: int,
                                inv_global_batch: Optional[float] = None, finish_flags: int = 0, optimizer=None,
                                companion=None, metrics_acc: Optional[torch.Tensor] = None) -> None:
        inv = 1.0 / batch if inv_global_batch is None else inv_global_batch
        dst = self.g_pred(batch)
        if not (g_pred.data_ptr() == dst.data_ptr() and g_pred.shape == dst.shape and g_pred.stride() == dst.stride()):
            dst.copy_(g_pred)
        self.backward(row_idx, row0, batch, seed, step, inv, finish_flags=finish_flags, optimizer=optimizer, companion=companion,
                      metrics_acc=metrics_acc)

    def mi_sandwich_bounds(self, enc_out: torch.Tensor, seed: int, step: int, feature: int):
        rows = mi_sandwich_rows(self.lib, self.device, self.to_device(enc_out), seed, step, feature)
        m = rows.mean(dim=1).cpu().numpy()
        return float(m[0]), float(m[1])

    def eps(self, row_idx, row0: int, batch: int, seed: int, step: int) -> torch.Tensor:
        out = torch.empty((batch, self.F, self.E), dtype=torch.float32, device=self.device)
        check(self.lib.dib_philox_normal_fill(_ptr(out), _ptr(row_idx), int(row0), batch, self.F, self.E, int(seed),
                                              int(step) & 0xFFFFFFFF, self._stream()), "dib_philox_normal_fill")
        return out


PROFILE_CATEGORIES = 19


def profile_summary(lib) -> dict:
    ms = (ctypes.c_double * PROFILE_CATEGORIES)()
    cnt = (c_int * PROFILE_CATEGORIES)()
    check(lib.dib_profile_summary_n(ms, cnt, PROFILE_CATEGORIES), "dib_profile_summary_n")
    bk = lambda mode, ni, nj: 64 if (ni, nj) == (2, 2) or (mode, ni, nj) == (2, 1, 2) else 32
    names = [f"dib_gemm_kernel<{mode}, {ni}, {nj}, {bk(mode, ni, nj)}>"
             for mode in (0, 1, 2) for ni in (1, 2) for nj in (1, 2)]
    names += ["dib_fused_encoder_fwd_kernel", "dib_fused_encoder_bwd_kernel", "other", "dib_attn_fwd_kernel", "dib_attn_bwd_kernel"]
    names += ["dib_wgrad_stream_kernel<4>", "dib_wgrad_stream_kernel<2>"]
    return {n: (float(ms[i]), int(cnt[i])) for i, n in enumerate(names) if cnt[i]}
```

### include/dib_hip.h

```cpp
#ifndef DIB_HIP_H
#define DIB_HIP_H

#include <stdint.h>

#ifdef __cplusplus
extern "C" {
#endif

typedef struct dib_layout dib_layout;
typedef void* dib_stream_t;

#define DIB_OK 0
#define DIB_E_ARG (-1)
#define DIB_E_SHAPE (-2)
#define DIB_E_WORKSPACE (-3)
#define DIB_E_UNSUPPORTED (-4)
#define DIB_E_NODEVICE (-5)

enum { DIB_ACT_LINEAR = 0, DIB_ACT_RELU = 1, DIB_ACT_LEAKY_RELU = 2, DIB_ACT_TANH = 3,
       DIB_ACT_SIGMOID = 4, DIB_ACT_ELU = 5, DIB_ACT_SOFTPLUS = 6 };

enum { DIB_LOSS_BCE_LOGITS = 0, DIB_LOSS_BCE = 1, DIB_LOSS_SPARSE_CCE_LOGITS = 2, DIB_LOSS_MSE = 3 };

enum { DIB_WS_U = 0,
       DIB_WS_PRED = 1,
       DIB_WS_ENC_OUT = 2,
       DIB_WS_G_U = 3,
       DIB_WS_STEP_OUT = 4,
       DIB_WS_G_PRED = 5,
       DIB_WS_ENC_H0 = 16,
       DIB_WS_INT_H0 = 32    };

const char* dib_version(void);
#define DIB_ABI_VERSION 7
int dib_abi_version(void);
const char* dib_error_string(int code);

int dib_layout_create(int num_features, const int* feature_dims, int n_enc_layers, const int* enc_units,
                      int embedding_dim, int n_int_layers, const int* int_units, int output_dim,
                      int use_positional_encoding, int n_freq, int activation, int output_activation,
                      dib_layout** out);
void dib_layout_destroy(dib_layout* l);
int64_t dib_layout_param_count(const dib_layout* l);
int dib_layout_param_block(const dib_layout* l, int net, int layer, int feature, int what, int64_t* offset,
                           int* rows, int* cols);
int64_t dib_layout_table_bytes(const dib_layout* l);
int dib_layout_upload_tables(dib_layout* l, void* dev_tables, dib_stream_t stream);
int dib_layout_set_step_counter(dib_layout* l, const uint32_t* step_dev);
int64_t dib_workspace_bytes(const dib_layout* l, int batch);
int dib_workspace_init(const dib_layout* l, int batch, void* ws, dib_stream_t stream);
int64_t dib_workspace_offset(const dib_layout* l, int batch, int which);
int dib_layout_wgrad_splits(const dib_layout* l, int batch);

#define DIB_FWD_DETERMINISTIC 1
#define DIB_FWD_INFERENCE 2
#define DIB_FWD_DEFER_SUMS 4
int dib_encoder_bank_fwd(dib_layout* l, const float* x, int64_t ldx, const int32_t* row_idx, int64_t row0,
                         int batch, const float* params, uint64_t seed, uint32_t step, int deterministic,
                         void* ws, dib_stream_t stream);
int dib_integration_fwd(dib_layout* l, int batch, const float* params, void* ws, dib_stream_t stream);

#define DIB_HEAD_DEFER_SUMS 1
#define DIB_HEAD_NO_GRAD 2
#define DIB_HEAD_DEFER_WGRAD 4
int dib_loss_fwd_bwd(dib_layout* l, int loss_kind, const float* y, int64_t ldy, const int32_t* row_idx,
                     int64_t row0, int batch, float inv_global_batch, int flags, void* ws, dib_stream_t stream);
int dib_integration_bwd(dib_layout* l, int batch, const float* params, float* grads, void* ws,
                        dib_stream_t stream);
int dib_output_head_fused_supported(const dib_layout* l, int loss_kind);
int dib_integration_fwd_hidden(dib_layout* l, int batch, const float* params, void* ws, dib_stream_t stream);
int dib_output_head_fused(dib_layout* l, int loss_kind, const float* y, int64_t ldy, const int32_t* row_idx, int64_t row0,
                          int batch, float inv_global_batch, int flags, const float* params, float* grads, void* ws,
                          dib_stream_t stream);
int dib_integration_bwd_hidden(dib_layout* l, int batch, const float* params, float* grads, void* ws,
                               dib_stream_t stream);
int dib_integration_head_step(dib_layout* l, int loss_kind, const float* y, int64_t ldy, const int32_t* row_idx, int64_t row0,
                              int batch, float inv_global_batch, int flags, const float* params, float* grads, void* ws,
                              dib_stream_t stream);
#define DIB_BWD_INTEGRATION_DONE 1
int dib_backward(dib_layout* l, int batch, const float* params, float* grads, const float* beta_dev, float inv_global_batch,
                 int flags, void* ws, dib_stream_t stream);
int dib_encoder_bank_bwd(dib_layout* l, int batch, const float* params, float* grads, const float* beta_dev,
                         float inv_global_batch, void* ws, dib_stream_t stream);
int dib_encoder_bank_bwd_stage(dib_layout* l, int batch, const float* params, float* grads, const float* beta_dev,
                               float inv_global_batch, int stage, void* ws, dib_stream_t stream);
int dib_grads_finalize(dib_layout* l, int batch, float* grads, void* ws, dib_stream_t stream);
int dib_grads_finalize_part(dib_layout* l, int batch, int part, float* grads, void* ws, dib_stream_t stream);
int dib_layout_part_range(const dib_layout* l, int part, int64_t* offset, int64_t* count);
int dib_metrics_accumulate(dib_layout* l, int batch, const float* beta_dev, float inv_global_batch,
                           float* metrics_acc, void* ws, dib_stream_t stream);
#define DIB_TAIL_FINALIZE 1
#define DIB_TAIL_KL 2
#define DIB_TAIL_LOSS 4
#define DIB_TAIL_ADAM 8
#define DIB_TAIL_BUMP 16
#define DIB_TAIL_METRICS 32
#define DIB_TAIL_SGD 64
#define DIB_TAIL_HEAD_WGRAD 128
#define DIB_TAIL_LOSS_HEAD 256
int dib_step_tail(dib_layout* l, int batch, int part, int flags, float* params, float* grads, float* adam_m, float* adam_v,
                  const float* lr_dev, int64_t* t_dev, float beta1, float beta2, float eps, float grad_scale,
                  const float* beta_dev, float inv_global_batch, float* metrics_acc, void* ws, dib_stream_t stream);

int dib_set_tuning(const char* key, int value);
int dib_get_tuning(const char* key, int* value);

int dib_adam_step(float* params, const float* grads, float* m, float* v, int64_t n, const float* lr_dev,
                  int64_t* t_dev, float beta1, float beta2, float eps, float grad_scale, dib_stream_t stream);
int dib_sgd_step(float* params, const float* grads, int64_t n, const float* lr_dev, float grad_scale,
                 dib_stream_t stream);
#define DIB_SYNC_WORDS 1056
int dib_reduce_adam_step(const float* partial, int nsplit, int64_t stride, float* params, float* grads, float* adam_m,
                         float* adam_v, int64_t n, const float* lr_dev, int64_t* t_dev, float beta1, float beta2, float eps,
                         float grad_scale, uint32_t* sync, dib_stream_t stream);

int dib_encode_deterministic(dib_layout* l, int feature, const float* x_f, int n, const float* params,
                             float* out, void* ws, dib_stream_t stream);
int dib_bhattacharyya(const float* mu1, const float* lv1, int n, const float* mu2, const float* lv2, int m,
                      int dim, float* out, dib_stream_t stream);
int64_t dib_infonce_workspace_bytes(int batch);
int dib_infonce_fwd_bwd(const float* emb_x, const float* emb_y, int batch, int dim, int similarity, float temperature,
                        float* g_x, float* g_y, float* loss_out, void* ws, dib_stream_t stream);
int dib_positional_encoding(const float* x, int64_t ldx, int n, int d, int n_freq, float* out, dib_stream_t stream);
int dib_positional_encoding_rows(const float* x, int64_t ldx, const int32_t* row_idx, int n, int d, int n_freq, float* out,
                                 dib_stream_t stream);

typedef struct dib_mlp_desc {
  int64_t w_off[4], b_off[4];
  int32_t n_hidden, width[4];
  int32_t in_dim, n_freq, act;
} dib_mlp_desc;
int dib_mlp_small_supported(const dib_mlp_desc* d, int batch);
int dib_mlp_small_fwd(const dib_mlp_desc* d, const float* params, const float* x, int64_t ldx, const int32_t* row_idx, int n,
                      float* a0, float* const* h, float* out, dib_stream_t stream);
int dib_mlp_small_bwd(const dib_mlp_desc* d, const float* params, const float* g_out, float* const* h, float* const* g, int n,
                      dib_stream_t stream);
int dib_mlp_small_head_supported(const dib_mlp_desc* d, int n);
int64_t dib_mlp_small_head_workspace_bytes(const dib_mlp_desc* d, int n);
int dib_mlp_small_head_step(const dib_mlp_desc* d, const float* params, const float* x, int n, const float* y, int64_t ldy,
                            int loss_kind, float inv_global_batch, float* const* h, float* const* g, float* pred, float* g_pred,
                            float* g_x, float* grads, float* sums3, void* ws, dib_stream_t stream);
int dib_integration_fwd_and_mlp_fwd(dib_layout* l, int batch, const float* params, void* ws, const dib_mlp_desc* d,
                                    const float* mlp_params, const float* x, int64_t ldx, const int32_t* row_idx, int n, float* a0,
                                    float* const* h, float* out, dib_stream_t stream);
int dib_backward_and_mlp_bwd(dib_layout* l, int batch, const float* params, float* grads, const float* beta_dev,
                             float inv_global_batch, int flags, void* ws, const dib_mlp_desc* d, const float* mlp_params,
                             const float* g_out, float* const* h, float* const* g, int n, dib_stream_t stream);

int64_t dib_mi_workspace_bytes(int n, int embedding_dim);
int dib_mi_sandwich_rows(const float* enc_out, int n, int embedding_dim, uint64_t seed, uint32_t step,
                         uint32_t feature, double* lower_rows, double* upper_rows, void* ws, dib_stream_t stream);
int dib_philox_normal_fill(float* eps, const int32_t* row_idx, int64_t row0, int batch, int num_features,
                           int embedding_dim, uint64_t seed, uint32_t step, dib_stream_t stream);
float dib_philox_normal_ref(uint64_t seed, uint32_t step, uint32_t row, uint32_t feature, uint32_t e);

int64_t dib_launch_count(void);
#define DIB_PROFILE_CATEGORIES 17
int dib_profile_enable(int on);
int dib_profile_summary(double* ms_by_category , int* launches_by_category );
#define DIB_PROFILE_CATEGORIES_N 19
int dib_profile_summary_n(double* ms_by_category , int* launches_by_category , int n);

int dib_gemm(int mode, int M, int N, int K, const float* A, int lda, const float* B, int ldb, float* C,
             int ldc, const float* bias, const float* aux, int ldaux, int act, void* dev_desc ,
             dib_stream_t stream);

#ifdef __cplusplus
}
#endif
#endif
```

Measured before the change: 8.363 million samples/s.

## Recompute first encoder hidden layer inside layer-2 weight-gradient kernel instead of stashing it

The fused encoder forward no longer writes the first hidden activation (h1) to HBM. The layer-2 weight-gradient GEMM now rebuilds each 32-row h1 tile on the fly from the positional-encoded inputs, W1 and b1 using extra MFMAs interleaved with the main accumulation. The aim is to remove the h1 store in the forward pass and its reload in the backward pass, a large f32 buffer at batch 65536. The cost is extra MFMA work and register pressure in the wgrad kernel, and a host-side materialize path for callers that still read h1.

```diff
diff --git a/distributed-information-bottleneck.github.io_amd/_lib.py b/distributed-information-bottleneck.github.io_amd/_lib.py
--- a/distributed-information-bottleneck.github.io_amd/_lib.py
+++ b/distributed-information-bottleneck.github.io_amd/_lib.py
@@ -85,6 +85,8 @@
     "dib_workspace_init": (c_int, [c_void_p, c_int, c_void_p, c_void_p]),
     "dib_workspace_offset": (c_int64, [c_void_p, c_int, c_int]),
     "dib_layout_wgrad_splits": (c_int, [c_void_p, c_int]),
+    "dib_workspace_h1_stashed": (c_int, [c_void_p, c_void_p]),
+    "dib_workspace_h1_materialize": (c_int, [c_void_p, c_int, c_void_p, c_void_p, c_void_p]),
     "dib_encoder_bank_fwd": (c_int, [c_void_p, c_void_p, c_int64, c_void_p, c_int64, c_int, c_void_p, c_uint64,
                                      c_uint32, c_int, c_void_p, c_void_p]),
     "dib_integration_fwd": (c_int, [c_void_p, c_int, c_void_p, c_void_p, c_void_p]),
diff --git a/distributed-information-bottleneck.github.io_amd/csrc/dib_api.hip b/distributed-information-bottleneck.github.io_amd/csrc/dib_api.hip
--- a/distributed-information-bottleneck.github.io_amd/csrc/dib_api.hip
+++ b/distributed-information-bottleneck.github.io_amd/csrc/dib_api.hip
@@ -18,6 +18,7 @@
 #include "dib_wgrad_stream.h"
 #include "dib_infonce_mfma.h"
 #include "dib_fused.h"
+#include "dib_wgrad_recompute.h"
 #include "dib_tail.h"
 #include "dib_small.h"
 #include "dib_st.h"
diff --git a/distributed-information-bottleneck.github.io_amd/csrc/dib_wgrad_recompute.h b/distributed-information-bottleneck.github.io_amd/csrc/dib_wgrad_recompute.h
--- /dev/null
+++ b/distributed-information-bottleneck.github.io_amd/csrc/dib_wgrad_recompute.h
@@ -0,0 +1,235 @@
+#pragma once
+#include "dib_fused.h"
+#include "dib_wgrad_stream.h"
+
+struct DibWgradH1Side {
+  long long p_boff;
+  long long w1_off;
+  long long b1_off;
+  int in_dim;
+  int act;
+};
+
+template <int NT, typename FBV>
+__device__ __forceinline__ void dib_wgh_bias_block(FBV& xc, const FBV (&rb)[4]) {
+  FBV y = xc;
+#pragma unroll
+  for (int t = 0; t < 4; ++t) y += rb[t];
+#pragma unroll
+  for (int u = 0; u < NT; ++u) y[u] = dib_wgs_swap_halves(y[u]);
+#pragma unroll
+  for (int t = 0; t < 4; ++t) y += rb[t];
+#pragma unroll
+  for (int u = 0; u < NT; ++u) xc[u] = dib_wgs_swap_halves(y[u]);
+}
+
+template <int NT, int CH, typename FBV>
+__device__ __forceinline__ void dib_wgh_epilogue(const DibGemmGroup& g, const dib_f32x16 (&acc)[4][NT], const FBV (&x)[CH],
+                                                 float* __restrict__ Cbase, float* __restrict__ bias_out, int batch, int slab,
+                                                 long long split_stride, int m0, int n0, int tm, int l31, int h) {
+  const long long coff = g.c_off + g.c_boff * batch + (long long)slab * split_stride;
+  float* Cg = Cbase + coff;
+  const bool vecC = ((coff | (long long)g.ldc) & (NT - 1)) == 0;
+#pragma unroll
+  for (int i = 0; i < 4; ++i) {
+#pragma unroll
+    for (int r = 0; r < 16; ++r) {
+      const int m = m0 + 4 * ((r & 3) + 8 * (r >> 2) + 4 * h) + i;
+      float* cp = Cg + (long long)m * g.ldc + n0 + NT * l31;
+      FBV v;
+#pragma unroll
+      for (int u = 0; u < NT; ++u) v[u] = acc[i][u][r];
+      if (vecC) {
+        *reinterpret_cast<FBV*>(cp) = v;
+      } else {
+#pragma unroll
+        for (int u = 0; u < NT; ++u) cp[u] = v[u];
+      }
+    }
+  }
+  if (bias_out != nullptr && g.bias_off >= 0 && tm == 0 && h == 0) {
+    FBV s = x[0];
+#pragma unroll
+    for (int c = 1; c < CH; ++c) s += x[c];
+    float* bp = bias_out + g.bias_off + (long long)slab * split_stride + n0 + NT * l31;
+#pragma unroll
+    for (int u = 0; u < NT; ++u) bp[u] = s[u];
+  }
+}
+
+__device__ __forceinline__ void dib_wgh_mfma_step(dib_f32x16 (&nxt)[4], float p, const float (&w)[4]) {
+  asm volatile("s_nop 1\n\t"
+               "v_mfma_f32_32x32x2_f32 %0, %4, %5, %0\n\t"
+               "v_mfma_f32_32x32x2_f32 %1, %4, %6, %1\n\t"
+               "v_mfma_f32_32x32x2_f32 %2, %4, %7, %2\n\t"
+               "v_mfma_f32_32x32x2_f32 %3, %4, %8, %3"
+               : "+v"(nxt[0]), "+v"(nxt[1]), "+v"(nxt[2]), "+v"(nxt[3])
+               : "v"(p), "v"(w[0]), "v"(w[1]), "v"(w[2]), "v"(w[3]));
+}
+__device__ __forceinline__ void dib_wgh_settle(dib_f32x16 (&nxt)[4]) {
+  asm volatile("s_nop 15\n\ts_nop 15" : "+v"(nxt[0]), "+v"(nxt[1]), "+v"(nxt[2]), "+v"(nxt[3]));
+}
+
+template <int CH, bool NTL, bool RELU>
+__global__ void __launch_bounds__(256, 1)
+dib_wgrad_h1_kernel(const DibGemmGroup* __restrict__ groups, const DibWgradH1Side* __restrict__ side,
+                    const float* __restrict__ Pbase, const float* __restrict__ params, const float* __restrict__ Bbase,
+                    float* __restrict__ Cbase, float* __restrict__ bias_out, int batch, int count, int tiles_m, int tiles_n,
+                    int nsplit, int rows_per_split, long long split_stride) {
+  static_assert(CH == 2 || CH == 4, "the tiled kernels' bias chains");
+  static_assert(kWgsGroups == 4, "one recomputed 32-row tile = one trip around a ring of four 8-row blocks");
+  constexpr int G = kWgsGroups, NT = 4;
+  typedef float f4v __attribute__((ext_vector_type(4)));
+  const int lane = threadIdx.x & 63, l31 = lane & 31, h = lane >> 5;
+  const int wave = __builtin_amdgcn_readfirstlane((int)(threadIdx.x >> 6));
+  const unsigned wid = blockIdx.x * 4u + (unsigned)wave;
+  const unsigned tiles = (unsigned)(tiles_m * tiles_n);
+  if (wid >= tiles * (unsigned)count * (unsigned)nsplit) return;
+  const int tile = (int)(wid % tiles);
+  const int grp = (int)((wid / tiles) % (unsigned)count), slab = (int)(wid / (tiles * (unsigned)count));
+  const int tm = tile / tiles_n, tn = tile % tiles_n;
+  const DibGemmGroup g = groups[grp];
+  const DibWgradH1Side sd = side[grp];
+  const int M = g.M < 0 ? batch : g.M;
+  const int N = g.N < 0 ? batch : g.N;
+  const int K = g.K < 0 ? batch : g.K;
+  const int m0 = tm * 128, n0 = tn * 128;
+  if (m0 >= M || n0 >= N) return;
+  const int kbeg = slab * rows_per_split;
+  const int nblk = max(0, min(K, kbeg + rows_per_split) - kbeg) >> 3;
+  const int ntile = nblk >> 2;
+
+  const char* uB = reinterpret_cast<const char*>(Bbase + g.b_off + g.b_boff * batch + (long long)kbeg * g.ldb + n0);
+  const unsigned rowB = (unsigned)g.ldb * 4u;
+  int lh = h, ll = l31;
+
+  const int in_dim = sd.in_dim;
+  float w1[4][4];
+#pragma unroll
+  for (int t = 0; t < 4; ++t) {
+    const int k = 4 * h + t;
+    const float* W1 = params + sd.w1_off + (long long)min(k, in_dim - 1) * M + m0 + 4 * l31;
+#pragma unroll
+    for (int u = 0; u < 4; ++u) w1[t][u] = (k < in_dim) ? W1[u] : 0.f;
+  }
+  const char* ub1 = reinterpret_cast<const char*>(params + sd.b1_off + m0);
+  float b1v[4];
+  auto load_b1 = [&](int u) { b1v[u] = *reinterpret_cast<const float*>(ub1 + 4 * u + (size_t)((unsigned)(4 * ll) * 4u)); };
+#pragma unroll
+  for (int u = 0; u < 4; ++u) load_b1(u);
+  const char* uP = reinterpret_cast<const char*>(Pbase + sd.p_boff * batch + (long long)kbeg * in_dim);
+  const unsigned rowsP = 32u * (unsigned)in_dim * 4u;
+  auto load_p = [&](int T, int t, float (&dst)[4]) {
+    const unsigned off = (unsigned)(ll * in_dim + min(4 * lh + t, in_dim - 1)) * 4u;
+    dst[t] = *reinterpret_cast<const float*>(uP + (size_t)((unsigned)T * rowsP) + (size_t)off);
+  };
+  auto mask_p = [&](float (&p)[4]) {
+#pragma unroll
+    for (int t = 0; t < 4; ++t) p[t] = (4 * lh + t < in_dim) ? p[t] : 0.f;
+  };
+  const float slope = dib_neg_slope(sd.act);
+  auto act_tile = [&](dib_f32x16& v) { dib_act_tile<RELU>(slope, v); };
+
+  dib_f32x16 acc[4][NT];
+#pragma unroll
+  for (int i = 0; i < 4; ++i)
+#pragma unroll
+    for (int j = 0; j < NT; ++j)
+#pragma unroll
+      for (int r = 0; r < 16; ++r) acc[i][j][r] = 0.f;
+
+  f4v x[CH];
+#pragma unroll
+  for (int c = 0; c < CH; ++c) x[c] = 0.f;
+
+  f4v rb[G][4];
+  auto load_step = [&](int slot, int blk, int t) {
+    const unsigned laneB = (unsigned)(4 * lh) * rowB + (unsigned)(NT * ll) * 4u;
+    const f4v* pb = reinterpret_cast<const f4v*>(uB + (size_t)((unsigned)(8 * blk + t) * rowB) + (size_t)laneB);
+    if (NTL) rb[slot][t] = __builtin_nontemporal_load(pb);
+    else rb[slot][t] = *pb;
+  };
+
+  float cur[4][16];
+  dib_f32x16 nxt[4];
+  float pn[4];
+  if (nblk > 0) {
+    float p0[4];
+#pragma unroll
+    for (int t = 0; t < 4; ++t) {
+      load_p(0, t, p0);
+      load_p(1, t, pn);
+    }
+    __builtin_amdgcn_sched_barrier(0);
+#pragma unroll
+    for (int j = 0; j < G - 1; ++j)
+#pragma unroll
+      for (int t = 0; t < 4; ++t) {
+        load_step(j, j, t);
+        __builtin_amdgcn_sched_barrier(0);
+      }
+    mask_p(p0);
+#pragma unroll
+    for (int u = 0; u < 4; ++u)
+#pragma unroll
+      for (int r = 0; r < 16; ++r) nxt[u][r] = b1v[u];
+#pragma unroll
+    for (int t = 0; t < 4; ++t) {
+      dib_wgh_mfma_step(nxt, p0[t], w1[t]);
+    }
+    dib_wgh_settle(nxt);
+#pragma unroll
+    for (int u = 0; u < 4; ++u) {
+      act_tile(nxt[u]);
+#pragma unroll
+      for (int r = 0; r < 16; ++r) cur[u][r] = nxt[u][r];
+    }
+  }
+#pragma unroll 1
+  for (int q0 = 0; q0 < nblk; q0 += G) {
+    const int Tnn = min((q0 >> 2) + 2, ntile - 1);
+    asm volatile("" : "+v"(lh), "+v"(ll));
+    mask_p(pn);
+#pragma unroll
+    for (int u = 0; u < 4; ++u)
+#pragma unroll
+      for (int r = 0; r < 16; ++r) nxt[u][r] = b1v[u];
+#pragma unroll
+    for (int j = 0; j < G; ++j) {
+      const int pf = min(q0 + j + G - 1, nblk - 1);
+#pragma unroll
+      for (int t = 0; t < 4; ++t) {
+        const f4v b = rb[j][t];
+#pragma unroll
+        for (int i = 0; i < 4; ++i)
+#pragma unroll
+          for (int u = 0; u < NT; ++u) acc[i][u] = DIB_MFMA(cur[i][4 * j + t], b[u], acc[i][u]);
+        if (j == 0) dib_wgh_mfma_step(nxt, pn[t], w1[t]);
+        __builtin_amdgcn_sched_barrier(0);
+        if (j == 2 && t == 0) {
+#pragma unroll
+          for (int u = 0; u < 4; ++u) load_b1(u);
+        }
+        load_step((j + G - 1) % G, pf, t);
+        if (j == 1) load_p(Tnn, t, pn);
+        __builtin_amdgcn_sched_barrier(0);
+      }
+      dib_wgh_bias_block<NT>(x[CH == 2 ? 0 : j], rb[j]);
+      if (j >= 1) {
+#pragma unroll
+        for (int u = 0; u < 4; ++u) {
+          if (j == 1) act_tile(nxt[u]);
+#pragma unroll
+          for (int r = (j == 1 ? 0 : 4 * j); r < 4 * j + 4; ++r) cur[u][r] = nxt[u][r];
+        }
+      }
+    }
+    if (CH == 2) {
+      const f4v s = x[0];
+      x[0] = x[1];
+      x[1] = s;
+    }
+  }
+
+  dib_wgh_epilogue<NT, CH>(g, acc, x, Cbase, bias_out, batch, slab, split_stride, m0, n0, tm, l31, h);
+}
diff --git a/distributed-information-bottleneck.github.io_amd/csrc/host/common.h b/distributed-information-bottleneck.github.io_amd/csrc/host/common.h
--- a/distributed-information-bottleneck.github.io_amd/csrc/host/common.h
+++ b/distributed-information-bottleneck.github.io_amd/csrc/host/common.h
@@ -17,6 +17,7 @@
 }
 
 constexpr int kProfCats = 19;
+constexpr int kProfWgradH1Part = 19;
 constexpr int kProfFusedFwd = 12, kProfFusedBwd = 13, kProfOther = 14, kProfAttnFwd = 15, kProfAttnBwd = 16;
 constexpr int kProfWgradStream128 = 17, kProfWgradStream64 = 18;
 struct Prof {
@@ -24,6 +25,7 @@
   std::mutex mu;
   std::vector<hipEvent_t> pool;
   std::vector<std::pair<hipEvent_t, hipEvent_t>> spans[kProfCats];
+  std::vector<size_t> h1_spans;
   hipEvent_t get() {
     if (!pool.empty()) { hipEvent_t e = pool.back(); pool.pop_back(); return e; }
     hipEvent_t e = nullptr;
@@ -34,14 +36,20 @@
 
 struct ProfScope {
   int cat; hipStream_t st; hipEvent_t a = nullptr, b = nullptr;
-  ProfScope(int c, hipStream_t s) : cat(c), st(s) {
+  bool h1_part;
+  ProfScope(int c, hipStream_t s, bool h1 = false) : cat(c), st(s), h1_part(h1) {
     if (g_prof.on.load(std::memory_order_relaxed) && cat != 14) {
       { std::lock_guard<std::mutex> lk(g_prof.mu); a = g_prof.get(); b = g_prof.get(); }
       (void)hipEventRecord(a, st);
     }
   }
   ~ProfScope() {
-    if (a) { (void)hipEventRecord(b, st); std::lock_guard<std::mutex> lk(g_prof.mu); g_prof.spans[cat].push_back({a, b}); }
+    if (a) {
+      (void)hipEventRecord(b, st);
+      std::lock_guard<std::mutex> lk(g_prof.mu);
+      if (h1_part) g_prof.h1_spans.push_back(g_prof.spans[cat].size());
+      g_prof.spans[cat].push_back({a, b});
+    }
   }
 };
 
@@ -66,6 +74,7 @@
   int wgrad_stream = 1;
   int wgrad_stream_rows = 8192;
   int wgrad_stream_fill = 85;
+  int wgrad_recompute_h1 = 1;
   int attn_fwd_waves = 8;
   int int_cluster_short_exchange = 1;
   int int_cluster = 8;
@@ -130,6 +139,7 @@
   if (!std::strcmp(key, "wgrad_stream")) return &t.wgrad_stream;
   if (!std::strcmp(key, "wgrad_stream_rows")) return &t.wgrad_stream_rows;
   if (!std::strcmp(key, "wgrad_stream_fill")) return &t.wgrad_stream_fill;
+  if (!std::strcmp(key, "wgrad_recompute_h1")) return &t.wgrad_recompute_h1;
   if (!std::strcmp(key, "wgrad_max_splits")) return &t.wgrad_max_splits;
   if (!std::strcmp(key, "num_cus")) return &t.num_cus;
   if (!std::strcmp(key, "attn_fwd_waves")) return &t.attn_fwd_waves;
@@ -181,6 +191,7 @@
     for (auto& sp : g_prof.spans[c]) { g_prof.pool.push_back(sp.first); g_prof.pool.push_back(sp.second); }
     g_prof.spans[c].clear();
   }
+  g_prof.h1_spans.clear();
   g_prof.on = on != 0;
   return DIB_OK;
 }
@@ -202,6 +213,18 @@
     launches_by_category[c] = (int)g_prof.spans[c].size();
   }
   for (int c = kProfCats; c < n; ++c) { ms_by_category[c] = 0.0; launches_by_category[c] = 0; }
+  if (n > kProfWgradH1Part) {
+    double tot = 0.0;
+    for (size_t i : g_prof.h1_spans) {
+      const auto& sp = g_prof.spans[kProfWgradStream128][i];
+      float ms = 0.f;
+      hipError_t e = hipEventElapsedTime(&ms, sp.first, sp.second);
+      if (e != hipSuccess) return (int)e;
+      tot += ms;
+    }
+    ms_by_category[kProfWgradH1Part] = tot;
+    launches_by_category[kProfWgradH1Part] = (int)g_prof.h1_spans.size();
+  }
   return DIB_OK;
 }
 
diff --git a/distributed-information-bottleneck.github.io_amd/csrc/host/encoder.h b/distributed-information-bottleneck.github.io_amd/csrc/host/encoder.h
--- a/distributed-information-bottleneck.github.io_amd/csrc/host/encoder.h
+++ b/distributed-information-bottleneck.github.io_amd/csrc/host/encoder.h
@@ -13,6 +13,30 @@
   for (int f = 0; f < l->F; ++f)
     if (l->in_dim[f] > 15) return false;
   return true;
+}
+
+static bool use_small_enc(const dib_layout* l, int batch);
+static dib_layout::H1Plan h1_recompute_plan(const dib_layout* l, const dib_layout::WsMap& m, const float* w, int batch) {
+  dib_layout::H1Plan r;
+  if (!knobs().wgrad_recompute_h1 || l->fused_id != 0 || !fused_bwd_ok(l) || l->h1_side.empty() || !l->dev_h1_side) return r;
+  if (use_small_enc(l, batch)) return r;
+  const GemmCall& c = l->enc_wgrad[1];
+  WgradStreamPlan sp;
+  if (!wgrad_stream_plan(l->table.data() + c.first, c, w + m.enc_h[0], w + m.g_enc_h[1], batch, m.nsplit, m.rows_per_split,
+                         true, m.nsplit, &sp) || sp.nt != 4)
+    return r;
+  r.recompute = true; r.ch = sp.ch; r.nsplit = sp.nsplit; r.rows_per_split = sp.rows_per_split;
+  return r;
+}
+static void h1_plan_record(const dib_layout* l, const void* ws, const dib_layout::H1Plan& p) {
+  std::lock_guard<std::mutex> lk(l->wg_mu);
+  if (p.recompute) l->h1_plan[ws] = p;
+  else l->h1_plan.erase(ws);
+}
+static dib_layout::H1Plan h1_plan_of(const dib_layout* l, const void* ws) {
+  std::lock_guard<std::mutex> lk(l->wg_mu);
+  auto it = l->h1_plan.find(ws);
+  return it == l->h1_plan.end() ? dib_layout::H1Plan() : it->second;
 }
 
 static int fused_encoder_fwd(dib_layout* l, const dib_layout::WsMap& m, float* w, const float* x, int64_t ldx,
@@ -28,6 +52,11 @@
   a.h2mask = (unsigned long long*)(w + m.h2mask);
   a.h1mask = fused_bwd_ok(l) ? (unsigned long long*)(w + m.h1mask) : nullptr;
   if (deterministic & DIB_FWD_INFERENCE) { a.h1 = nullptr; a.h2 = nullptr; a.h2mask = nullptr; a.h1mask = nullptr; }
+  else {
+    const dib_layout::H1Plan plan = h1_recompute_plan(l, m, w, batch);
+    h1_plan_record(l, w, plan);
+    if (plan.recompute) a.h1 = nullptr;
+  }
   a.step_dev = l->step_dev;
   const int gx = fused_gx(l, batch);
   *gx_out = gx;
@@ -168,6 +197,18 @@
     const float* gout = last ? w + m.dout : w + m.g_enc_h[ly];
     const float* hin = ly == 0 ? w + m.P : w + m.enc_h[ly - 1];
     const bool wgrad_here = (last ? (stages & 2) : (stages & 1)) && !(fused && ly == 0);
+    if (wgrad_here && ly == 1 && fused && !small) {
+      const dib_layout::H1Plan plan = h1_plan_of(l, ws);
+      if (plan.recompute) {
+        const GemmCall& c = l->enc_wgrad[ly];
+        rc = launch_wgrad_h1(plan.ch, l->act == 1, l->dev_groups, l->dev_h1_side, c, w + m.P, params, gout, gt, gt, batch, plan.nsplit,
+                             plan.rows_per_split, sstride, st);
+        if (rc == DIB_OK && m.nsplit > 1)
+          rc = retire_stale_slabs(l, batch, l->table.data() + c.first, c.count, plan.nsplit, m.nsplit, gt, sstride, st);
+        if (rc) return rc;
+        continue;
+      }
+    }
     if (wgrad_here) {
       const bool halve = l->enc_wgrad[ly].max_n <= 64 && m.nsplit >= 32 && (m.nsplit % 2) == 0;
       rc = launch_gemm<2>(l, l->enc_wgrad[ly], hin, gout, gt, nullptr, nullptr, gt, batch, 0,
@@ -195,6 +236,7 @@
   const auto m = l->map(batch);
   float* w = (float*)ws;
   if (use_small_enc(l, batch)) {
+    if (!(deterministic & DIB_FWD_INFERENCE)) h1_plan_record(l, ws, dib_layout::H1Plan());
     int rc = small_encoder_fwd(l, m, w, x, ldx, row_idx, row0, batch, params, seed, step, deterministic, st);
     if (rc || (deterministic & DIB_FWD_DEFER_SUMS)) return rc;
     ProfScope ps(kProfOther, st);
@@ -245,6 +287,15 @@
                                float inv_global_batch, int stage, void* ws, dib_stream_t stream) {
   if (stage != 1 && stage != 2) return DIB_E_ARG;
   return encoder_bank_bwd_stages(l, batch, params, grads, beta_dev, inv_global_batch, stage, ws, stream);
+}
+
+int dib_workspace_h1_materialize(dib_layout* l, int batch, const float* params, void* ws, dib_stream_t stream) {
+  if (!l || !params || !ws || batch <= 0 || l->n_enc < 1) return DIB_E_ARG;
+  if (!l->dev_groups) return DIB_E_WORKSPACE;
+  const auto m = l->map(batch);
+  float* w = (float*)ws;
+  return launch_gemm<0>(l, l->enc_fwd[0], w + m.P, params, w + m.enc_h[0], params, nullptr, nullptr, batch, l->act, 1, 0, 0,
+                        (hipStream_t)stream);
 }
 
 int dib_encode_deterministic(dib_layout* l, int feature, const float* x_f, int n, const float* params, float* out,
diff --git a/distributed-information-bottleneck.github.io_amd/csrc/host/gemm.h b/distributed-information-bottleneck.github.io_amd/csrc/host/gemm.h
--- a/distributed-information-bottleneck.github.io_amd/csrc/host/gemm.h
+++ b/distributed-information-bottleneck.github.io_amd/csrc/host/gemm.h
@@ -91,6 +91,63 @@
   *rps_out = brps;
 }
 
+static void wgrad_tile_rule(int M, int N, int nsplit, int count, bool* ni1, bool* nj1) {
+  *ni1 = M <= 64;
+  *nj1 = N <= 64;
+  if (!*ni1 && !*nj1) {
+    const long long wgs = (long long)cdiv(M, 128) * cdiv(N, 128) * nsplit * count;
+    if (wgs < 256) *ni1 = true;
+    if (*ni1 && !*nj1 && (long long)cdiv(M, 64) * cdiv(N, 128) * nsplit * count < 128) *nj1 = true;
+  }
+}
+
+struct WgradStreamPlan { int nt = 0, ch = 0, nsplit = 0, rows_per_split = 0; };
+static bool wgrad_stream_plan(const DibGemmGroup* host_groups, const GemmCall& c, const float* A, const float* B, int batch, int nsplit,
+                              int rows_per_split, bool auto_split, int max_splits, WgradStreamPlan* plan) {
+  const int M = c.max_m < 0 ? batch : c.max_m, N = c.max_n < 0 ? batch : c.max_n;
+  int nt = 0;
+  if (c.count <= 0 || !wgrad_stream_shape_ok(host_groups, c.count, batch, A, B, &nt)) return false;
+  int ns = nsplit, rps = rows_per_split;
+  const long long tiles = (long long)cdiv(M, 128) * cdiv(N, 32 * nt) * c.count;
+  if (auto_split && ns > 1 && knobs().split_policy)
+    pick_wgrad_splits(tiles, split_rule_cus() * kWgradStreamWavesPerCu, batch, std::max(ns, max_splits), &ns, &rps);
+  if (!wgrad_stream_slabs_ok(host_groups, c.count, batch, tiles, ns, rps)) return false;
+  bool ni1, nj1;
+  wgrad_tile_rule(M, N, nsplit, c.count, &ni1, &nj1);
+  plan->nt = nt;
+  plan->ch = nt == 2 || nj1 ? 4 : 2;
+  plan->nsplit = ns;
+  plan->rows_per_split = rps;
+  return true;
+}
+
+template <int CH, bool RELU>
+int launch_wgrad_h1_t(const DibGemmGroup* dev_groups, const DibWgradH1Side* dev_side, const GemmCall& c, int M, int N, const float* P,
+                      const float* params, const float* B, float* C, float* bias_out, int batch, int nsplit, int rows_per_split,
+                      long long split_stride, hipStream_t st) {
+  const int tm = cdiv(M, 128), tn = cdiv(N, 128);
+  const long long waves = (long long)tm * tn * c.count * nsplit;
+  if (waves >= (1ll << 31)) return DIB_E_UNSUPPORTED;
+  ProfScope ps(kProfWgradStream128, st, true);
+  const dim3 grid((unsigned)((waves + 3) / 4));
+  if ((long long)nsplit * rows_per_split >= knobs().stream_rows)
+    DIB_LAUNCH((dib_wgrad_h1_kernel<CH, true, RELU>), grid, dim3(256), 0, st, dev_groups + c.first, dev_side, P, params, B, C,
+               bias_out, batch, c.count, tm, tn, nsplit, rows_per_split, split_stride);
+  else
+    DIB_LAUNCH((dib_wgrad_h1_kernel<CH, false, RELU>), grid, dim3(256), 0, st, dev_groups + c.first, dev_side, P, params, B, C,
+               bias_out, batch, c.count, tm, tn, nsplit, rows_per_split, split_stride);
+  return (int)hipGetLastError();
+}
+static int launch_wgrad_h1(int ch, bool relu, const DibGemmGroup* dev_groups, const DibWgradH1Side* dev_side, const GemmCall& c,
+                           const float* P, const float* params, const float* B, float* C, float* bias_out, int batch, int nsplit,
+                           int rows_per_split, long long split_stride, hipStream_t st) {
+#define DIB_GO(CH, RELU) launch_wgrad_h1_t<CH, RELU>(dev_groups, dev_side, c, c.max_m, c.max_n, P, params, B, C, bias_out, batch, nsplit, \
+                                                     rows_per_split, split_stride, st)
+  if (ch == 4) return relu ? DIB_GO(4, true) : DIB_GO(4, false);
+  return relu ? DIB_GO(2, true) : DIB_GO(2, false);
+#undef DIB_GO
+}
+
 template <int MODE>
 int launch_gemm(const DibGemmGroup* dev_groups, const GemmCall& c, const float* A, const float* B, float* C,
                 const float* bias, const float* aux, float* bias_out, int batch, int act, int nsplit, int rows_per_split,
@@ -106,24 +163,15 @@
     if (wgs < knobs().fwd_small_wgs) ni1 = true;
     if (ni1 && !nj1 && (long long)cdiv(M, 64) * cdiv(N, 128) * c.count < (MODE == 0 ? knobs().fwd_narrow_wgs : 128)) nj1 = true;
   }
-  if (MODE == 2 && !ni1 && !nj1) {
-    const long long wgs = (long long)cdiv(M, 128) * cdiv(N, 128) * nsplit * c.count;
-    if (wgs < 256) ni1 = true;
-    if (ni1 && !nj1 && (long long)cdiv(M, 64) * cdiv(N, 128) * nsplit * c.count < 128) nj1 = true;
-  }
+  if (MODE == 2) wgrad_tile_rule(M, N, nsplit, c.count, &ni1, &nj1);
   if constexpr (MODE == 2) {
-    int nt = 0;
-    if (wgrad_stream_shape_ok(host_groups, c.count, batch, A, B, &nt)) {
-      int ns = nsplit, rps = rows_per_split;
-      const long long tiles = (long long)cdiv(M, 128) * cdiv(N, 32 * nt) * c.count;
-      if (auto_split && ns > 1 && knobs().split_policy)
-        pick_wgrad_splits(tiles, split_rule_cus() * kWgradStreamWavesPerCu, batch, std::max(ns, max_splits), &ns, &rps);
-      if (wgrad_stream_slabs_ok(host_groups, c.count, batch, tiles, ns, rps)) {
-        if (ns_used) *ns_used = ns;
-        if (nt == 2) return launch_wgrad_stream<2, 4>(dev_groups, c, M, N, A, B, C, bias_out, batch, ns, rps, split_stride, st);
-        return nj1 ? launch_wgrad_stream<4, 4>(dev_groups, c, M, N, A, B, C, bias_out, batch, ns, rps, split_stride, st)
-                   : launch_wgrad_stream<4, 2>(dev_groups, c, M, N, A, B, C, bias_out, batch, ns, rps, split_stride, st);
-      }
+    WgradStreamPlan sp;
+    if (wgrad_stream_plan(host_groups, c, A, B, batch, nsplit, rows_per_split, auto_split, max_splits, &sp)) {
+      const int ns = sp.nsplit, rps = sp.rows_per_split;
+      if (ns_used) *ns_used = ns;
+      if (sp.nt == 2) return launch_wgrad_stream<2, 4>(dev_groups, c, M, N, A, B, C, bias_out, batch, ns, rps, split_stride, st);
+      return sp.ch == 4 ? launch_wgrad_stream<4, 4>(dev_groups, c, M, N, A, B, C, bias_out, batch, ns, rps, split_stride, st)
+                        : launch_wgrad_stream<4, 2>(dev_groups, c, M, N, A, B, C, bias_out, batch, ns, rps, split_stride, st);
     }
   }
   if (MODE == 2 && auto_split && nsplit > 1 && knobs().split_policy) {
diff --git a/distributed-information-bottleneck.github.io_amd/csrc/host/layout.h b/distributed-information-bottleneck.github.io_amd/csrc/host/layout.h
--- a/distributed-information-bottleneck.github.io_amd/csrc/host/layout.h
+++ b/distributed-information-bottleneck.github.io_amd/csrc/host/layout.h
@@ -44,6 +44,10 @@
   std::vector<int4> featmap;
   const long long* dev_fused_offs = nullptr;
   const int4* dev_featmap = nullptr;
+  struct H1Plan { bool recompute = false; int ch = 2, nsplit = 0, rows_per_split = 0; };
+  std::vector<DibWgradH1Side> h1_side;
+  const DibWgradH1Side* dev_h1_side = nullptr;
+  mutable std::map<const void*, H1Plan> h1_plan;
   const unsigned* step_dev = nullptr;
   bool sb_enc = false, sb_int = false;
   int sb_int_lds = 0;
@@ -281,6 +285,16 @@
     for (int ly = LE; ly < 3; ++ly)
       for (int f = 0; f < F; ++f) l->fused_offs.push_back(0);
     for (int f = 0; f < F; ++f) l->featmap.push_back(make_int4(l->dims[f], l->in_dim[f], l->x_off[f], l->in_off[f]));
+    bool in8 = true;
+    for (int f = 0; f < F; ++f) in8 = in8 && l->in_dim[f] <= 8;
+    if (l->fused_id == 0 && in8)
+      for (int f = 0; f < F; ++f) {
+        DibWgradH1Side sd;
+        std::memset(&sd, 0, sizeof(sd));
+        sd.p_boff = l->in_off[f]; sd.w1_off = l->enc_w_off[0][f]; sd.b1_off = l->enc_b_off[0][f];
+        sd.in_dim = l->in_dim[f]; sd.act = act;
+        l->h1_side.push_back(sd);
+      }
   }
   {
     bool in_ok = true;
@@ -338,7 +352,8 @@
   return align_up((int64_t)l->table.size() * sizeof(DibGemmGroup), 256) +
          align_up((int64_t)l->colmap.size() * sizeof(int4), 256) +
          align_up((int64_t)l->fused_offs.size() * sizeof(long long), 256) +
-         align_up((int64_t)l->featmap.size() * sizeof(int4), 256);
+         align_up((int64_t)l->featmap.size() * sizeof(int4), 256) +
+         align_up((int64_t)l->h1_side.size() * sizeof(DibWgradH1Side), 256);
 }
 
 int dib_layout_upload_tables(dib_layout* l, void* dev_tables, dib_stream_t stream) {
@@ -361,6 +376,12 @@
   l->dev_colmap = (const int4*)cm;
   l->dev_fused_offs = (const long long*)fo;
   l->dev_featmap = (const int4*)fmp;
+  if (!l->h1_side.empty()) {
+    char* hs = fmp + align_up((int64_t)l->featmap.size() * sizeof(int4), 256);
+    e = hipMemcpyAsync(hs, l->h1_side.data(), l->h1_side.size() * sizeof(DibWgradH1Side), hipMemcpyHostToDevice, st);
+    if (e != hipSuccess) return (int)e;
+    l->dev_h1_side = (const DibWgradH1Side*)hs;
+  }
   return DIB_OK;
 }
 
@@ -378,6 +399,7 @@
 int dib_workspace_init(const dib_layout* l, int batch, void* ws, dib_stream_t stream) {
   if (!l || !ws || batch <= 0) return DIB_E_ARG;
   const auto m = l->map(batch);
+  { std::lock_guard<std::mutex> lk(l->wg_mu); l->h1_plan.erase(ws); }
   hipError_t e0 = hipMemsetAsync((float*)ws + m.sync, 0, (size_t)DIB_TAIL_SYNC_WORDS * sizeof(unsigned), (hipStream_t)stream);
   if (e0 != hipSuccess) return (int)e0;
   if (l->sb_int && batch <= kSmallMaxBatch) {
@@ -416,6 +438,13 @@
   return o * (int64_t)sizeof(float);
 }
 
+int dib_workspace_h1_stashed(const dib_layout* l, const void* ws) {
+  if (!l || !ws) return DIB_E_ARG;
+  std::lock_guard<std::mutex> lk(l->wg_mu);
+  auto it = l->h1_plan.find(ws);
+  return it == l->h1_plan.end() || !it->second.recompute ? 1 : 0;
+}
+
 int dib_layout_wgrad_splits(const dib_layout* l, int batch) {
   if (!l || batch <= 0) return DIB_E_ARG;
   return l->map(batch).nsplit;
diff --git a/distributed-information-bottleneck.github.io_amd/engine.py b/distributed-information-bottleneck.github.io_amd/engine.py
--- a/distributed-information-bottleneck.github.io_amd/engine.py
+++ b/distributed-information-bottleneck.github.io_amd/engine.py
@@ -420,6 +420,14 @@
 
     def enc_h(self, batch: int, layer: int) -> torch.Tensor:
         w = self.enc_units[layer]
+        if layer == 0 and int(self.lib.dib_workspace_h1_stashed(self.layout, _ptr(self.workspace(batch)))) == 0:
+            rc = int(self.lib.dib_workspace_h1_materialize(self.layout, batch, _ptr(self.params), _ptr(self.workspace(batch)),
+                                                           self._stream()))
+            if rc != 0:
+                raise _lib.DibError(f"enc_h(layer=0): the last forward of batch size {batch} did not stash the first hidden layer (its "
+                                    f"layer-2 weight gradient recomputes it) and it could not be recomputed here "
+                                    f"(dib_workspace_h1_materialize -> {rc}); dib_set_tuning('wgrad_recompute_h1', 0) before the "
+                                    f"forward keeps the stash")
         return self.ws_view(batch, _lib.WS_ENC_H0 + layer, batch * self.F * w).view(self.F, batch, w)
 
     def int_h(self, batch: int, layer: int) -> torch.Tensor:
diff --git a/include/dib_hip.h b/include/dib_hip.h
--- a/include/dib_hip.h
+++ b/include/dib_hip.h
@@ -51,6 +51,8 @@
 int dib_workspace_init(const dib_layout* l, int batch, void* ws, dib_stream_t stream);
 int64_t dib_workspace_offset(const dib_layout* l, int batch, int which);
 int dib_layout_wgrad_splits(const dib_layout* l, int batch);
+int dib_workspace_h1_stashed(const dib_layout* l, const void* ws);
+int dib_workspace_h1_materialize(dib_layout* l, int batch, const float* params, void* ws, dib_stream_t stream);
 
 #define DIB_FWD_DETERMINISTIC 1
 #define DIB_FWD_INFERENCE 2
@@ -158,7 +160,7 @@
 #define DIB_PROFILE_CATEGORIES 17
 int dib_profile_enable(int on);
 int dib_profile_summary(double* ms_by_category , int* launches_by_category );
-#define DIB_PROFILE_CATEGORIES_N 19
+#define DIB_PROFILE_CATEGORIES_N 20
 int dib_profile_summary_n(double* ms_by_category , int* launches_by_category , int n);
 
 int dib_gemm(int mode, int M, int N, int K, const float* A, int lda, const float* B, int ldb, float* C,
```

Measured after the change: 8.664 million samples/s (median of 6 runs). 3.6% higher.
